# selkies-project/selkies

Hardware: AMD Instinct MI355X
Metric: encoded_fps_1080p60_h264 (higher is better)
Workload: dtype uint8; 1 GPU; model=hipflux h264enc-striped (HIP gfx950), global_batch=1, seq_len=2073600, parallelism=sessions1, resolution=1920x1080, qp=28, content=noise, pipeline=hip-h264, pipeline_depth=2

## Files before the change

native/hip/h264_deblock.hip:

```cpp
#include <hip/hip_runtime.h>

#include <type_traits>

#include "h264_gpu_layout.h"
#include "h264_kernels.h"

namespace hipflux {
namespace h264gpu {

__constant__ uint8_t cDbAlpha[52] = {
    0, 0, 0, 0, 0, 0, 0, 0, 0, 0, 0, 0, 0, 0, 0, 0,
    4, 4, 5, 6, 7, 8, 9, 10, 12, 13, 15, 17, 20, 22, 25, 28,
    32, 36, 40, 45, 50, 56, 63, 71, 80, 90, 101, 113, 127, 144,
    162, 182, 203, 226, 255, 255};
__constant__ uint8_t cDbBeta[52] = {
    0, 0, 0, 0, 0, 0, 0, 0, 0, 0, 0, 0, 0, 0, 0, 0,
    2, 2, 2, 3, 3, 3, 3, 4, 4, 4, 6, 6, 7, 7, 8, 8,
    9, 9, 10, 10, 11, 11, 12, 12, 13, 13, 14, 14, 15, 15,
    16, 16, 17, 17, 18, 18};
__constant__ uint8_t cDbTc0[52][3] = {
    {0,0,0},{0,0,0},{0,0,0},{0,0,0},{0,0,0},{0,0,0},{0,0,0},{0,0,0},
    {0,0,0},{0,0,0},{0,0,0},{0,0,0},{0,0,0},{0,0,0},{0,0,0},{0,0,0},
    {0,0,0},{0,0,1},{0,0,1},{0,0,1},{0,0,1},{0,1,1},{0,1,1},{1,1,1},
    {1,1,1},{1,1,1},{1,1,1},{1,1,2},{1,1,2},{1,1,2},{1,1,2},{1,2,3},
    {1,2,3},{2,2,3},{2,2,4},{2,3,4},{2,3,4},{3,3,5},{3,4,6},{3,4,6},
    {4,5,7},{4,5,8},{5,6,9},{6,7,10},{6,8,11},{7,9,12},{8,10,13},
    {9,12,15},{10,13,17},{11,16,20},{13,18,23},{14,20,25}};

__constant__ int cDbChromaQp[52] = {
    0, 1, 2, 3, 4, 5, 6, 7, 8, 9, 10, 11, 12, 13, 14, 15, 16, 17, 18,
    19, 20, 21, 22, 23, 24, 25, 26, 27, 28, 29, 29, 30, 31, 32, 32, 33,
    34, 34, 35, 35, 36, 36, 37, 37, 37, 38, 38, 38, 39, 39, 39, 39};

__device__ __forceinline__ int db_clip3d(int lo, int hi, int v) {
  return v < lo ? lo : v > hi ? hi : v;
}
__device__ __forceinline__ int db_clip8d(int v) {
  return v < 0 ? 0 : v > 255 ? 255 : v;
}

struct DbInfo {
  int intra;
  int mvx, mvy;
  unsigned nz;
};

__device__ __forceinline__ int db_bs_d(const DbInfo& mp, int pblk,
                                       const DbInfo& mq, int qblk,
                                       bool mb_edge) {
  if (mp.intra || mq.intra) return mb_edge ? 4 : 3;
  if (((mp.nz >> pblk) & 1) || ((mq.nz >> qblk) & 1)) return 2;
  if (abs(mp.mvx - mq.mvx) >= 4 || abs(mp.mvy - mq.mvy) >= 4) return 1;
  return 0;
}

__device__ void db_luma_line(uint8_t* e, int st, int bs, int alpha,
                             int beta, int tc0) {
  const int p0 = e[-st], p1 = e[-2 * st], p2 = e[-3 * st], p3 = e[-4 * st];
  const int q0 = e[0], q1 = e[st], q2 = e[2 * st], q3 = e[3 * st];
  if (abs(p0 - q0) >= alpha || abs(p1 - p0) >= beta ||
      abs(q1 - q0) >= beta)
    return;
  const bool ap = abs(p2 - p0) < beta;
  const bool aq = abs(q2 - q0) < beta;
  if (bs < 4) {
    const int tc = tc0 + (ap ? 1 : 0) + (aq ? 1 : 0);
    const int delta =
        db_clip3d(-tc, tc, ((q0 - p0) * 4 + (p1 - q1) + 4) >> 3);
    e[-st] = (uint8_t)db_clip8d(p0 + delta);
    e[0] = (uint8_t)db_clip8d(q0 - delta);
    if (ap)
      e[-2 * st] = (uint8_t)(p1 + db_clip3d(-tc0, tc0,
                       (p2 + ((p0 + q0 + 1) >> 1) - 2 * p1) >> 1));
    if (aq)
      e[st] = (uint8_t)(q1 + db_clip3d(-tc0, tc0,
                  (q2 + ((p0 + q0 + 1) >> 1) - 2 * q1) >> 1));
  } else {
    const bool small = abs(p0 - q0) < ((alpha >> 2) + 2);
    if (ap && small) {
      e[-st] = (uint8_t)((p2 + 2 * p1 + 2 * p0 + 2 * q0 + q1 + 4) >> 3);
      e[-2 * st] = (uint8_t)((p2 + p1 + p0 + q0 + 2) >> 2);
      e[-3 * st] = (uint8_t)((2 * p3 + 3 * p2 + p1 + p0 + q0 + 4) >> 3);
    } else {
      e[-st] = (uint8_t)((2 * p1 + p0 + q1 + 2) >> 2);
    }
    if (aq && small) {
      e[0] = (uint8_t)((q2 + 2 * q1 + 2 * q0 + 2 * p0 + p1 + 4) >> 3);
      e[st] = (uint8_t)((q2 + q1 + q0 + p0 + 2) >> 2);
      e[2 * st] = (uint8_t)((2 * q3 + 3 * q2 + q1 + q0 + p0 + 4) >> 3);
    } else {
      e[0] = (uint8_t)((2 * q1 + q0 + p1 + 2) >> 2);
    }
  }
}

__device__ void db_chroma_line(uint8_t* e, int st, int bs, int alpha,
                               int beta, int tc0) {
  const int p0 = e[-st], p1 = e[-2 * st];
  const int q0 = e[0], q1 = e[st];
  if (abs(p0 - q0) >= alpha || abs(p1 - p0) >= beta ||
      abs(q1 - q0) >= beta)
    return;
  if (bs < 4) {
    const int tc = tc0 + 1;
    const int delta =
        db_clip3d(-tc, tc, ((q0 - p0) * 4 + (p1 - q1) + 4) >> 3);
    e[-st] = (uint8_t)db_clip8d(p0 + delta);
    e[0] = (uint8_t)db_clip8d(q0 - delta);
  } else {
    e[-st] = (uint8_t)((2 * p1 + p0 + q1 + 2) >> 2);
    e[0] = (uint8_t)((2 * q1 + q0 + p1 + 2) >> 2);
  }
}

struct DbShared {
  uint8_t y[16][kMaxSegMbw * 16];
  uint8_t cb[8][kMaxSegMbw * 8];
  uint8_t cr[8][kMaxSegMbw * 8];
  DbInfo info[kMaxSegMbw];
};

struct DbSharedMono {
  uint8_t y[16][kMaxSegMbw * 16];
  DbInfo info[kMaxSegMbw];
};

template <bool MONO>
__device__ __forceinline__ void deblock_body(
    uint8_t* __restrict__ curY, uint8_t* __restrict__ curCb,
    uint8_t* __restrict__ curCr, int ypitch, int cpitch, int mbw,
    const RowJob& job, const int16_t* __restrict__ levels,
    const int* __restrict__ meta) {
  __shared__ std::conditional_t<MONO, DbSharedMono, DbShared> sh;
  if (job.flags & kJobIdr) {
  }
  const int lane = threadIdx.x;
  const int segw = job.seg_mbw;
  const int y0 = job.mb_row * 16, cy0 = job.mb_row * 8;
  const int px0 = job.mbx0 * 16, cpx0 = job.mbx0 * 8;
  const int wpx = segw * 16, cwpx = segw * 8;

  for (int r = 0; r < 16; ++r)
    for (int x = lane; x < wpx; x += 64)
      sh.y[r][x] = curY[(size_t)(y0 + r) * ypitch + px0 + x];
  if constexpr (!MONO) {
    for (int r = 0; r < 8; ++r)
      for (int x = lane; x < cwpx; x += 64) {
        sh.cb[r][x] = curCb[(size_t)(cy0 + r) * cpitch + cpx0 + x];
        sh.cr[r][x] = curCr[(size_t)(cy0 + r) * cpitch + cpx0 + x];
      }
  }
  for (int m = lane; m < segw; m += 64) {
    const size_t mb = (size_t)job.mb_row * mbw + job.mbx0 + m;
    const int m0 = meta[mb * kMetaPerMb + 0];
    const int m1 = meta[mb * kMetaPerMb + 1];
    const int mode = m0 & 3;
    DbInfo di;
    di.intra = mode == kIntra || (job.flags & kJobIdr);
    di.mvx = mode == kInter ? (int)(short)(m1 & 0xFFFF) : 0;
    di.mvy = mode == kInter ? (m1 >> 16) : 0;
    di.nz = 0;
    if (!MONO && mode == kInter) {
      const int16_t* lv = levels + mb * kLevelsPerMb + kLumaAcOff;
      for (int b = 0; b < 16; ++b) {
        int any = 0;
        for (int i = 0; i < 16; ++i) any |= lv[b * 16 + i] != 0;
        di.nz |= (unsigned)any << b;
      }
    }
    sh.info[m] = di;
  }
  __syncthreads();

  const int qp = db_clip3d(0, 51, job.qp);
  const int qpc = cDbChromaQp[qp];
  const int alpha = cDbAlpha[qp], beta = cDbBeta[qp];
  const int alpha_c = cDbAlpha[qpc], beta_c = cDbBeta[qpc];

  for (int m = 0; m < segw; ++m) {
    const int x0 = m * 16, cx0 = m * 8;
    for (int e = 0; e < 4; ++e) {
      if (lane < 16) {
        if (!(e == 0 && m == 0)) {
          const int pblk = (lane >> 2) * 4 + (e == 0 ? 3 : e - 1);
          const int qblk = (lane >> 2) * 4 + e;
          const DbInfo& mp = e == 0 ? sh.info[m - 1] : sh.info[m];
          const int bs = db_bs_d(mp, pblk, sh.info[m], qblk, e == 0);
          if (bs) {
            const int tc0 = bs < 4 ? cDbTc0[qp][bs - 1] : 0;
            db_luma_line(&sh.y[lane][x0 + e * 4], 1, bs, alpha, beta,
                         tc0);
          }
        }
      } else if constexpr (MONO) {
      } else if (lane < 32 && e < 2) {
        if (!(e == 0 && m == 0)) {
          const int pl = (lane - 16) >> 3, yy = (lane - 16) & 7;
          const int lrow = (yy * 2) >> 2;
          const int pblk = lrow * 4 + (e == 0 ? 3 : 1);
          const int qblk = lrow * 4 + (e == 0 ? 0 : 2);
          const DbInfo& mp = e == 0 ? sh.info[m - 1] : sh.info[m];
          const int bs = db_bs_d(mp, pblk, sh.info[m], qblk, e == 0);
          if (bs) {
            const int tc0 = bs < 4 ? cDbTc0[qpc][bs - 1] : 0;
            uint8_t* base = pl ? &sh.cr[yy][cx0 + e * 4]
                               : &sh.cb[yy][cx0 + e * 4];
            db_chroma_line(base, 1, bs, alpha_c, beta_c, tc0);
          }
        }
      } else if (lane < 32 && e == 2) {
        const int pl = (lane - 16) >> 3, xx = (lane - 16) & 7;
        const int lcol = (xx * 2) >> 2;
        const int pblk = 1 * 4 + lcol;
        const int qblk = 2 * 4 + lcol;
        const int bs = db_bs_d(sh.info[m], pblk, sh.info[m], qblk, false);
        if (bs) {
          const int tc0 = bs < 4 ? cDbTc0[qpc][bs - 1] : 0;
          uint8_t* base = pl ? &sh.cr[4][cx0 + xx] : &sh.cb[4][cx0 + xx];
          db_chroma_line(base, kMaxSegMbw * 8, bs, alpha_c, beta_c, tc0);
        }
      }
      __syncthreads();
    }
    for (int e = 1; e < 4; ++e) {
      if (lane < 16) {
        const int pblk = (e - 1) * 4 + (lane >> 2);
        const int qblk = e * 4 + (lane >> 2);
        const int bs = db_bs_d(sh.info[m], pblk, sh.info[m], qblk, false);
        if (bs) {
          const int tc0 = bs < 4 ? cDbTc0[qp][bs - 1] : 0;
          db_luma_line(&sh.y[e * 4][x0 + lane], kMaxSegMbw * 16, bs,
                       alpha, beta, tc0);
        }
      }
      __syncthreads();
    }
  }

  for (int r = 0; r < 16; ++r)
    for (int x = lane; x < wpx; x += 64)
      curY[(size_t)(y0 + r) * ypitch + px0 + x] = sh.y[r][x];
  if constexpr (!MONO) {
    for (int r = 0; r < 8; ++r)
      for (int x = lane; x < cwpx; x += 64) {
        curCb[(size_t)(cy0 + r) * cpitch + cpx0 + x] = sh.cb[r][x];
        curCr[(size_t)(cy0 + r) * cpitch + cpx0 + x] = sh.cr[r][x];
      }
  }
}

__global__ __launch_bounds__(64) void k_h264_deblock(
    uint8_t* __restrict__ curY, uint8_t* __restrict__ curCb,
    uint8_t* __restrict__ curCr, int ypitch, int cpitch, int mbw,
    const RowJob* __restrict__ jobs, const int16_t* __restrict__ levels,
    const int* __restrict__ meta) {
  const RowJob job = jobs[blockIdx.x];
  deblock_body<false>(curY, curCb, curCr, ypitch, cpitch, mbw, job, levels,
                      meta);
}

__global__ __launch_bounds__(64) void k_h264_deblock_mono(
    uint8_t* __restrict__ cur, size_t plane_stride, int pitch, int mbw,
    const RowJob* __restrict__ jobs, const int* __restrict__ meta) {
  const RowJob job = jobs[blockIdx.x];
  deblock_body<true>(cur + (size_t)job.plane * plane_stride, nullptr,
                     nullptr, pitch, 0, mbw, job, nullptr,
                     meta + (size_t)job.mb_base * kMetaPerMb);
}

void launch_h264_deblock_mono(uint8_t* d_cur, size_t plane_stride, int pitch,
                              int mbw, int n_jobs, const RowJob* d_jobs,
                              const int* d_meta, hipStream_t stream) {
  if (n_jobs == 0) return;
  hipLaunchKernelGGL(k_h264_deblock_mono, dim3(n_jobs), dim3(64), 0, stream,
                     d_cur, plane_stride, pitch, mbw, d_jobs, d_meta);
}

void launch_h264_deblock(uint8_t* d_curY, uint8_t* d_curCb,
                         uint8_t* d_curCr, int ypitch, int cpitch, int mbw,
                         int n_jobs, const RowJob* d_jobs,
                         const int16_t* d_levels, const int* d_meta,
                         hipStream_t stream) {
  if (n_jobs == 0) return;
  hipLaunchKernelGGL(k_h264_deblock, dim3(n_jobs), dim3(64), 0, stream,
                     d_curY, d_curCb, d_curCr, ypitch, cpitch, mbw, d_jobs,
                     d_levels, d_meta);
}

}
}
```

native/hip/h264_kernels.h:

```cpp
#pragma once
#include <hip/hip_runtime.h>

#include <cstdint>

#include "h264_gpu_layout.h"

namespace hipflux {
namespace h264gpu {

void launch_downsample2(const uint8_t* src, int spitch, int sw, int sh,
                        uint8_t* dst, int dpitch, hipStream_t stream);

void launch_h264_me(const uint8_t* srcY, int ypitch, int w, int h,
                    const uint8_t* refY, const uint8_t* srcY2,
                    const uint8_t* refY2, int ypitch2, int mbw, int n_jobs,
                    const RowJob* d_jobs, int* d_meta, hipStream_t stream,
                    bool use_mfma = true);

void launch_h264_rows4(const uint8_t* srcY, const uint8_t* srcCb,
                       const uint8_t* srcCr, int ypitch, int cpitch, int w,
                       int h, const uint8_t* refY, const uint8_t* refCb,
                       const uint8_t* refCr, uint8_t* curY, uint8_t* curCb,
                       uint8_t* curCr, int mbw, int n_jobs,
                       const struct RowJob* d_jobs, int16_t* d_levels,
                       int* d_meta, hipStream_t stream);

void launch_h264_rows(const uint8_t* srcY, const uint8_t* srcCb,
                      const uint8_t* srcCr, int ypitch, int cpitch, int w,
                      int h, const uint8_t* refY, const uint8_t* refCb,
                      const uint8_t* refCr, uint8_t* curY, uint8_t* curCb,
                      uint8_t* curCr, int mbw, int n_jobs,
                      const RowJob* d_jobs, int16_t* d_levels, int* d_meta,
                      hipStream_t stream);

void launch_h264_deblock(uint8_t* d_curY, uint8_t* d_curCb,
                         uint8_t* d_curCr, int ypitch, int cpitch, int mbw,
                         int n_jobs, const RowJob* d_jobs,
                         const int16_t* d_levels, const int* d_meta,
                         hipStream_t stream);

void launch_h264_rows4_mono(const uint8_t* src, const uint8_t* ref,
                            uint8_t* cur, size_t plane_stride, int pitch,
                            int w, int h, int mbw, int n_jobs,
                            const RowJob* d_jobs, int16_t* d_levels,
                            int* d_meta, hipStream_t stream);

void launch_h264_deblock_mono(uint8_t* d_cur, size_t plane_stride, int pitch,
                              int mbw, int n_jobs, const RowJob* d_jobs,
                              const int* d_meta, hipStream_t stream);

void launch_h264_cavlc_mono(const int16_t* d_levels, const int* d_meta,
                            int mbw, int n_jobs, const RowJob* d_jobs,
                            uint32_t* d_stage, int* d_nbits, uint32_t* d_out,
                            int out_stride_words, int* d_out_bits,
                            hipStream_t stream);

void launch_h264_cavlc(const int16_t* d_levels, const int* d_meta, int mbw,
                       int n_jobs, const RowJob* d_jobs, uint32_t* d_stage,
                       int* d_nbits, uint32_t* d_out, int out_stride_words,
                       int* d_out_bits, hipStream_t stream);

}
}
```

native/module.cpp:

```cpp
#include <pybind11/functional.h>
#include <pybind11/numpy.h>
#include <pybind11/pybind11.h>
#include <pybind11/stl.h>

#include "audio.h"
#include "cpu/damage.h"
#include "cpu/h264/cavlc.h"
#include "cpu/h264/encoder.h"
#include "cpu/h264/seg_plan.h"
#include "cpu/hevc/cabac.h"
#include "cpu/hevc/encoder.h"
#include "cpu/opus/celt.h"
#include "cpu/opus/range_coder.h"
#include "cpu/jpeg_enc.h"
#include "cpu/overlay.h"
#include "cpu/scale.h"
#include "engine.h"
#include "frontend_hip.h"
#include <hip/hip_runtime.h>

#include "rccl_comm.h"

namespace py = pybind11;
using namespace hipflux;

namespace hipflux {
int hip_device_count();
}

PYBIND11_MODULE(_native, m) {
  m.doc() = "hipflux: MI355X-native capture+encode engine";

  py::class_<CaptureSettings>(m, "CaptureSettings")
      .def(py::init<>())
      .def_readwrite("capture_width", &CaptureSettings::capture_width)
      .def_readwrite("capture_height", &CaptureSettings::capture_height)
      .def_readwrite("capture_x", &CaptureSettings::capture_x)
      .def_readwrite("capture_y", &CaptureSettings::capture_y)
      .def_readwrite("target_fps", &CaptureSettings::target_fps)
      .def_readwrite("capture_cursor", &CaptureSettings::capture_cursor)
      .def_readwrite("output_mode", &CaptureSettings::output_mode)
      .def_readwrite("capture_scale", &CaptureSettings::capture_scale)
      .def_readwrite("capture_scale_div", &CaptureSettings::capture_scale_div)
      .def_readwrite("pipeline_depth", &CaptureSettings::pipeline_depth)
      .def_readwrite("video_fullframe", &CaptureSettings::video_fullframe)
      .def_readwrite("use_cpu", &CaptureSettings::use_cpu)
      .def_readwrite("gpu_id", &CaptureSettings::gpu_id)
      .def_readwrite("gpu_frontend", &CaptureSettings::gpu_frontend)
      .def_readwrite("video_bitrate_kbps", &CaptureSettings::video_bitrate_kbps)
      .def_readwrite("video_crf", &CaptureSettings::video_crf)
      .def_readwrite("video_cbr_mode", &CaptureSettings::video_cbr_mode)
      .def_readwrite("video_min_qp", &CaptureSettings::video_min_qp)
      .def_readwrite("video_max_qp", &CaptureSettings::video_max_qp)
      .def_readwrite("vbv_multiplier", &CaptureSettings::vbv_multiplier)
      .def_readwrite("keyframe_interval_s", &CaptureSettings::keyframe_interval_s)
      .def_readwrite("video_streaming_mode", &CaptureSettings::video_streaming_mode)
      .def_readwrite("video_deblock", &CaptureSettings::video_deblock)
      .def_readwrite("video_fullcolor", &CaptureSettings::video_fullcolor)
      .def_readwrite("use_paint_over_quality", &CaptureSettings::use_paint_over_quality)
      .def_readwrite("paint_over_trigger_frames", &CaptureSettings::paint_over_trigger_frames)
      .def_readwrite("video_paintover_crf", &CaptureSettings::video_paintover_crf)
      .def_readwrite("video_paintover_burst_frames", &CaptureSettings::video_paintover_burst_frames)
      .def_readwrite("damage_block_threshold", &CaptureSettings::damage_block_threshold)
      .def_readwrite("damage_block_duration", &CaptureSettings::damage_block_duration)
      .def_readwrite("jpeg_quality", &CaptureSettings::jpeg_quality)
      .def_readwrite("jpeg_paintover_quality", &CaptureSettings::jpeg_paintover_quality)
      .def_readwrite("stripe_height", &CaptureSettings::stripe_height)
      .def_readwrite("omit_stripe_headers", &CaptureSettings::omit_stripe_headers)
      .def_readwrite("watermark_path", &CaptureSettings::watermark_path)
      .def_readwrite("watermark_location", &CaptureSettings::watermark_location)
      .def_readwrite("capture_backend", &CaptureSettings::capture_backend)
      .def_readwrite("display", &CaptureSettings::display)
      .def_readwrite("recording_path", &CaptureSettings::recording_path)
      .def_readwrite("debug_logging", &CaptureSettings::debug_logging);

  py::class_<ScreenCapture>(m, "ScreenCapture")
      .def(py::init<>())
      .def(
          "start_capture",
          [](ScreenCapture& self, py::function cb, const CaptureSettings& s) {
            {
              py::gil_scoped_release rel;
              self.stop_capture();
            }
            self.clear_callback();
            StripeCallback native_cb = [cb](const EncodedStripe& st) {
              py::gil_scoped_acquire gil;
              try {
                py::bytes data(reinterpret_cast<const char*>(st.data),
                               st.size);
                cb(data, st.frame_id, st.y, st.width, st.height,
                   st.is_keyframe, st.capture_ts_ms, st.encode_done_ms,
                   static_cast<int>(st.type));
              } catch (py::error_already_set& e) {
                e.discard_as_unraisable("hipflux stripe callback");
              }
            };
            py::gil_scoped_release rel;
            self.start_capture(std::move(native_cb), s);
          },
          py::arg("callback"), py::arg("settings"),
          "Start the native capture+encode thread. callback(data, frame_id, "
          "y, width, height, is_keyframe, capture_ts_ms, encode_done_ms, "
          "stripe_type) runs on the native thread.")
      .def("stop_capture", &ScreenCapture::stop_capture,
           py::call_guard<py::gil_scoped_release>())
      .def(
          "set_cursor_callback",
          [](ScreenCapture& self, py::function cb) {
            self.clear_cursor_callback();
            self.set_cursor_callback(
                [cb](int w, int h, int hx, int hy, const uint32_t* argb,
                     size_t n) {
                  py::gil_scoped_acquire gil;
                  try {
                    cb(w, h, hx, hy,
                       py::bytes(reinterpret_cast<const char*>(argb),
                                 n * 4));
                  } catch (py::error_already_set& e) {
                    e.discard_as_unraisable("hipflux cursor callback");
                  }
                });
          },
          "callback(width, height, hot_x, hot_y, argb_bytes) on shape change")
      .def_property_readonly("is_capturing", &ScreenCapture::is_capturing)
      .def("request_idr_frame", &ScreenCapture::request_idr_frame)
      .def("update_framerate", &ScreenCapture::update_framerate)
      .def("update_video_bitrate", &ScreenCapture::update_video_bitrate)
      .def("update_crf", &ScreenCapture::update_crf)
      .def("update_jpeg_quality", &ScreenCapture::update_jpeg_quality)
      .def("update_vbv_multiplier", &ScreenCapture::update_vbv_multiplier)
      .def("update_capture_region", &ScreenCapture::update_capture_region)
      .def_property_readonly("frames_captured", &ScreenCapture::frames_captured)
      .def_property_readonly("frames_encoded", &ScreenCapture::frames_encoded)
      .def_property_readonly("stripes_emitted", &ScreenCapture::stripes_emitted)
      .def_property_readonly("last_encode_ms", &ScreenCapture::last_encode_ms)
      .def_property_readonly("last_frontend_ms",
                             &ScreenCapture::last_frontend_ms)
      .def_property_readonly("pipeline",
                             [](ScreenCapture& s) { return s.pipeline_name(); })
      .def_property_readonly("frontend",
                             [](ScreenCapture& s) { return s.frontend_name(); });

  m.def(
      "jpeg_encode",
      [](py::buffer bgrx, int width, int height, int quality, bool fullcolor) {
        py::buffer_info info = bgrx.request();
        if (info.size < static_cast<ssize_t>(width) * height * 4)
          throw std::runtime_error("buffer too small for WxHx4");
        std::vector<uint8_t> out;
        {
          py::gil_scoped_release rel;
          jpeg_encode_bgrx(static_cast<const uint8_t*>(info.ptr), width * 4,
                           width, height, quality, fullcolor, out);
        }
        return py::bytes(reinterpret_cast<const char*>(out.data()),
                         out.size());
      },
      py::arg("bgrx"), py::arg("width"), py::arg("height"),
      py::arg("quality") = 80, py::arg("fullcolor") = false,
      "Encode a BGRX buffer as baseline JPEG (CPU reference path).");

  m.def(
      "_jpeg_encode_restart",
      [](py::buffer bgrx, int width, int height, int quality,
         bool fullcolor) {
        py::buffer_info info = bgrx.request();
        std::vector<uint8_t> out;
        {
          py::gil_scoped_release rel;
          jpeg_encode_bgrx(static_cast<const uint8_t*>(info.ptr), width * 4,
                           width, height, quality, fullcolor, out, true);
        }
        return py::bytes(reinterpret_cast<const char*>(out.data()),
                         out.size());
      },
      py::arg("bgrx"), py::arg("width"), py::arg("height"),
      py::arg("quality") = 80, py::arg("fullcolor") = false,
      "Test hook: restart-row JPEG framing (the GPU entropy structure).");

  struct PyH264 {
    h264::StripeEncoder enc;
    int w, h, ypitch, cpitch;
    bool fullcolor;
    std::vector<uint8_t> yuv;
    PyH264(int width, int height, bool deblock, bool fc)
        : enc(width, height, deblock, fc), w(width), h(height),
          fullcolor(fc) {
      ypitch = (w + 15) & ~15;
      cpitch = fullcolor ? ypitch : ypitch / 2;
      int yh = (h + 15) & ~15;
      yuv.resize(static_cast<size_t>(ypitch) * yh * (fullcolor ? 3 : 2) *
                 (fullcolor ? 1 : 3) / (fullcolor ? 1 : 4));
    }
  };
  py::class_<PyH264>(m, "H264Encoder")
      .def(py::init<int, int, bool, bool>(), py::arg("width"),
           py::arg("height"), py::arg("deblock") = true,
           py::arg("fullcolor") = false)
      .def(
          "encode",
          [](PyH264& self, py::buffer bgrx, int qp, bool idr) {
            py::buffer_info info = bgrx.request();
            if (info.size < static_cast<ssize_t>(self.w) * self.h * 4)
              throw std::runtime_error("buffer too small");
            std::vector<uint8_t> out;
            h264::EncodeStats st;
            {
              py::gil_scoped_release rel;
              uint8_t* y = self.yuv.data();
              int yh = (self.h + 15) & ~15;
              uint8_t* cb = y + static_cast<size_t>(self.ypitch) * yh;
              uint8_t* cr = cb + static_cast<size_t>(self.cpitch) *
                                     (self.fullcolor ? yh : yh / 2);
              if (self.fullcolor)
                h264::bgrx_to_yuv444(static_cast<const uint8_t*>(info.ptr),
                                     self.w * 4, self.w, self.h, y, cb, cr,
                                     self.ypitch);
              else
                h264::bgrx_to_yuv420(static_cast<const uint8_t*>(info.ptr),
                                     self.w * 4, self.w, self.h, y,
                                     self.ypitch, cb, cr, self.cpitch);
              self.enc.encode_frame(y, self.ypitch, cb, cr, self.cpitch, qp,
                                    idr, out, &st);
            }
            py::dict d;
            d["data"] = py::bytes(reinterpret_cast<const char*>(out.data()),
                                  out.size());
            d["is_idr"] = st.is_idr;
            d["mb_intra"] = st.mb_intra;
            d["mb_inter"] = st.mb_inter;
            d["mb_skip"] = st.mb_skip;
            return d;
          },
          py::arg("bgrx"), py::arg("qp") = 26, py::arg("idr") = false)
      .def(
          "encode_yuv",
          [](PyH264& self, py::buffer ybuf, py::buffer cbbuf, py::buffer crbuf,
             int qp, bool idr) {
            auto yi = ybuf.request(), cbi = cbbuf.request(),
                 cri = crbuf.request();
            std::vector<uint8_t> out;
            h264::EncodeStats st;
            {
              py::gil_scoped_release rel;
              self.enc.encode_frame(static_cast<const uint8_t*>(yi.ptr),
                                    self.w, static_cast<const uint8_t*>(cbi.ptr),
                                    static_cast<const uint8_t*>(cri.ptr),
                                    (self.w + 1) / 2, qp, idr, out, &st);
            }
            return py::bytes(reinterpret_cast<const char*>(out.data()),
                             out.size());
          },
          py::arg("y"), py::arg("cb"), py::arg("cr"), py::arg("qp") = 26,
          py::arg("idr") = false,
          "Encode from tightly-packed YUV420 planes (pitch = width).")
      .def("recon",
           [](PyH264& self) {
             int yh = (self.h + 15) & ~15;
             int ch = self.fullcolor ? yh : yh / 2;
             py::bytes y(reinterpret_cast<const char*>(self.enc.recon_y()),
                         static_cast<size_t>(self.enc.recon_ypitch()) * yh);
             py::bytes cb(reinterpret_cast<const char*>(self.enc.recon_cb()),
                          static_cast<size_t>(self.enc.recon_cpitch()) * ch);
             py::bytes cr(reinterpret_cast<const char*>(self.enc.recon_cr()),
                          static_cast<size_t>(self.enc.recon_cpitch()) * ch);
             return py::make_tuple(y, cb, cr, self.enc.recon_ypitch(),
                                   self.enc.recon_cpitch());
           });

  struct PyHevc {
    hevc::StripeEncoder enc;
    int w, h, ypitch, cpitch;
    bool fullcolor;
    std::vector<uint8_t> yuv;
    PyHevc(int width, int height, int slices_per_row, bool fc)
        : enc(width, height, slices_per_row, fc), w(width), h(height),
          fullcolor(fc) {
      ypitch = (width + 15) & ~15;
      cpitch = fc ? ypitch : ypitch / 2;
      int yh = (height + 15) & ~15;
      yuv.resize(fc ? static_cast<size_t>(ypitch) * yh * 3
                    : static_cast<size_t>(ypitch) * yh * 3 / 2);
    }
  };
  py::class_<PyHevc>(m, "HevcEncoder")
      .def(py::init<int, int, int, bool>(), py::arg("width"),
           py::arg("height"), py::arg("slices_per_row") = 1,
           py::arg("fullcolor") = false)
      .def(
          "encode",
          [](PyHevc& self, py::buffer bgrx, int qp) {
            py::buffer_info info = bgrx.request();
            if (info.size < static_cast<ssize_t>(self.w) * self.h * 4)
              throw std::runtime_error("buffer too small");
            std::vector<uint8_t> out;
            hevc::EncodeStats st;
            {
              py::gil_scoped_release rel;
              uint8_t* y = self.yuv.data();
              int yh = (self.h + 15) & ~15;
              uint8_t* cb = y + static_cast<size_t>(self.ypitch) * yh;
              uint8_t* cr = cb + static_cast<size_t>(self.cpitch) *
                                     (self.fullcolor ? yh : yh / 2);
              if (self.fullcolor)
                h264::bgrx_to_yuv444(static_cast<const uint8_t*>(info.ptr),
                                     self.w * 4, self.w, self.h, y, cb, cr,
                                     self.ypitch);
              else
                h264::bgrx_to_yuv420(static_cast<const uint8_t*>(info.ptr),
                                     self.w * 4, self.w, self.h, y,
                                     self.ypitch, cb, cr, self.cpitch);
              self.enc.encode_frame(y, self.ypitch, cb, cr, self.cpitch, qp,
                                    out, &st);
            }
            py::dict d;
            d["data"] = py::bytes(reinterpret_cast<const char*>(out.data()),
                                  out.size());
            d["qp"] = st.frame_qp;
            d["ctus"] = st.ctu_count;
            return d;
          },
          py::arg("bgrx"), py::arg("qp") = 30)
      .def("recon", [](PyHevc& self) {
        int yh = (self.h + 15) & ~15;
        int yp = self.enc.recon_ypitch(), cp = self.enc.recon_cpitch();
        int chh = self.fullcolor ? yh : yh / 2;
        py::bytes y(reinterpret_cast<const char*>(self.enc.recon_y()),
                    static_cast<size_t>(yp) * yh);
        py::bytes cb(reinterpret_cast<const char*>(self.enc.recon_cb()),
                     static_cast<size_t>(cp) * chh);
        py::bytes cr(reinterpret_cast<const char*>(self.enc.recon_cr()),
                     static_cast<size_t>(cp) * chh);
        return py::make_tuple(y, cb, cr, yp, cp);
      });

  m.def(
      "_hevc_cabac_encode",
      [](const std::vector<std::tuple<int, int, int>>& ops, int qp) {
        std::vector<uint8_t> bytes;
        hevc::CabacEncoder cab(bytes);
        hevc::ContextBank bank;
        bank.init(qp);
        for (const auto& op : ops) {
          int kind = std::get<0>(op), ctx = std::get<1>(op),
              bin = std::get<2>(op);
          if (kind == 0)
            cab.encode_bin(bank.ctx[ctx % hevc::kNumContexts], bin);
          else if (kind == 1)
            cab.encode_bypass(bin);
          else
            cab.encode_terminate(bin);
        }
        auto tail = cab.finish();
        return py::make_tuple(
            py::bytes(reinterpret_cast<const char*>(bytes.data()),
                      bytes.size()),
            tail.bits, tail.nbits);
      },
      py::arg("ops"), py::arg("qp") = 30);

  py::class_<opus::CeltEncoder>(m, "OpusEncoder")
      .def(py::init<int>(), py::arg("bitrate_bps") = 96000)
      .def("set_bitrate", &opus::CeltEncoder::set_bitrate)
      .def(
          "encode",
          [](opus::CeltEncoder& e, py::buffer pcm, int channels) {
            py::buffer_info info = pcm.request();
            if (info.size <
                static_cast<ssize_t>(opus::kFrameSamples) * channels)
              throw std::runtime_error("need 960 frames of s16 PCM");
            std::vector<uint8_t> out;
            {
              py::gil_scoped_release rel;
              out = e.encode_frame(
                  static_cast<const int16_t*>(info.ptr), channels);
            }
            return py::bytes(reinterpret_cast<const char*>(out.data()),
                             out.size());
          },
          py::arg("pcm"), py::arg("channels") = 2);

  m.def("_opus_range_encode",
        [](const std::vector<std::tuple<int, int, int>>& ops,
           size_t capacity) {
          opus::RangeEncoder ec(capacity);
          static const uint8_t icdf4[4] = {200, 120, 40, 0};
          for (const auto& op : ops) {
            int kind = std::get<0>(op), a = std::get<1>(op),
                b = std::get<2>(op);
            if (kind == 0)
              ec.enc_bit_logp(a, static_cast<unsigned>(b));
            else if (kind == 1)
              ec.enc_uint(static_cast<uint32_t>(a),
                          static_cast<uint32_t>(b));
            else if (kind == 2)
              ec.enc_bits(static_cast<uint32_t>(a),
                          static_cast<unsigned>(b));
            else
              ec.enc_icdf(a % 4, icdf4, 8);
          }
          ec.done();
          auto s = ec.stream();
          return py::make_tuple(
              py::bytes(reinterpret_cast<const char*>(s.data()),
                        s.size()),
              ec.error());
        });

  py::class_<TileComm>(m, "TileComm")
      .def(py::init<int, int, const std::string&, int>(), py::arg("rank"),
           py::arg("world"), py::arg("uid"), py::arg("device") = 0)
      .def_static("make_uid",
                  [] { return py::bytes(TileComm::make_uid()); })
      .def_property_readonly("rank", &TileComm::rank)
      .def_property_readonly("world", &TileComm::world)
      .def(
          "exchange",
          [](TileComm& c, uintptr_t src_dev, size_t bytes, int schedule) {
            py::gil_scoped_release rel;
            return c.exchange(src_dev, bytes, schedule);
          },
          py::arg("src_dev"), py::arg("bytes"), py::arg("schedule") = 1,
          "All-gather this rank's device payload to every rank; "
          "schedule 0 = ring (bulk), 1 = one-hop p2p (latency). "
          "Returns ms.")
      .def(
          "exchange_host",
          [](TileComm& c, py::bytes payload, int schedule) {
            std::string s = payload;
            void* d = nullptr;
            if (hipMalloc(&d, s.size()) != hipSuccess)
              throw std::runtime_error("alloc failed");
            (void)hipMemcpy(d, s.data(), s.size(), hipMemcpyHostToDevice);
            double ms;
            {
              py::gil_scoped_release rel;
              ms = c.exchange(reinterpret_cast<uintptr_t>(d), s.size(),
                              schedule);
            }
            (void)hipFree(d);
            return ms;
          },
          py::arg("payload"), py::arg("schedule") = 1,
          "Upload host bytes and exchange (tests).")
      .def("gathered",
           [](TileComm& c, int rank, size_t bytes) {
             auto v = c.gathered(rank, bytes);
             return py::bytes(reinterpret_cast<const char*>(v.data()),
                              v.size());
           })
      .def(
          "broadcast",
          [](TileComm& c, uintptr_t buf, size_t bytes, int root) {
            py::gil_scoped_release rel;
            return c.broadcast(buf, bytes, root);
          },
          py::arg("buf_dev"), py::arg("bytes"), py::arg("root") = 0,
          "Broadcast a reference-frame buffer from root. Returns ms.");

  m.def(
      "bgrx_to_yuv420",
      [](py::buffer bgrx, int width, int height) {
        py::buffer_info info = bgrx.request();
        int cw = (width + 1) / 2, ch = (height + 1) / 2;
        std::vector<uint8_t> y(static_cast<size_t>(width) * height),
            cb(static_cast<size_t>(cw) * ch), cr(static_cast<size_t>(cw) * ch);
        h264::bgrx_to_yuv420(static_cast<const uint8_t*>(info.ptr), width * 4,
                             width, height, y.data(), width, cb.data(),
                             cr.data(), cw);
        return py::make_tuple(
            py::bytes(reinterpret_cast<char*>(y.data()), y.size()),
            py::bytes(reinterpret_cast<char*>(cb.data()), cb.size()),
            py::bytes(reinterpret_cast<char*>(cr.data()), cr.size()));
      },
      py::arg("bgrx"), py::arg("width"), py::arg("height"));

  m.def(
      "_pipeline_encode",
      [](const std::string& kind, py::list frames, int w, int h, int qp,
         int stripe_h, int output_mode, bool dump, bool fullcolor,
         int pipeline_depth, py::object encode_mask) -> py::object {
        const size_t n_stripes =
            stripe_h > 0 ? static_cast<size_t>((h + stripe_h - 1) / stripe_h)
                         : 0;
        std::vector<std::vector<bool>> mask;
        if (!encode_mask.is_none()) {
          if (!py::isinstance<py::list>(encode_mask))
            throw py::value_error("encode_mask must be a list of lists");
          py::list ml = encode_mask.cast<py::list>();
          if (ml.size() != frames.size())
            throw py::value_error("encode_mask needs one entry per frame");
          for (py::handle fm : ml) {
            if (!py::isinstance<py::list>(fm))
              throw py::value_error("encode_mask must be a list of lists");
            py::list fl = py::reinterpret_borrow<py::list>(fm);
            if (fl.size() != n_stripes)
              throw py::value_error(
                  "encode_mask entry needs one bool per stripe");
            std::vector<bool> row;
            for (py::handle b : fl) row.push_back(b.cast<bool>());
            mask.push_back(std::move(row));
          }
        }
        CaptureSettings s;
        s.capture_width = w;
        s.capture_height = h;
        s.output_mode = output_mode;
        s.stripe_height = stripe_h;
        s.video_crf = qp;
        s.jpeg_quality = qp;
        s.video_fullcolor = fullcolor;
        s.use_cpu = kind == "cpu";
        s.gpu_id = kind == "cpu" ? -1 : 0;
        std::unique_ptr<EncodePipeline> p;
        if (kind == "gpu") {
          p = make_hip_pipeline(s);
          if (!p) throw std::runtime_error("no HIP pipeline available");
        } else {
          p = output_mode == 1   ? make_cpu_h264_pipeline(s)
              : output_mode == 2 ? make_cpu_hevc_pipeline(s)
                                 : make_cpu_jpeg_pipeline(s);
        }
        p->set_pipeline_depth(pipeline_depth);
        std::vector<py::list> per_frame(frames.size());
        auto sink = [&](EncodedStripe& st) {
          per_frame[st.frame_id].append(py::make_tuple(
              py::bytes(reinterpret_cast<const char*>(st.data), st.size),
              st.y, st.height, st.is_keyframe));
        };
        py::list result;
        for (size_t i = 0; i < frames.size(); ++i) {
          py::buffer buf = frames[i].cast<py::buffer>();
          py::buffer_info info = buf.request();
          if (info.size < static_cast<ssize_t>(w) * h * 4)
            throw std::runtime_error("frame buffer too small");
          RawFrame f;
          f.data = static_cast<const uint8_t*>(info.ptr);
          f.width = w;
          f.height = h;
          f.stride = w * 4;
          f.ts_ms = now_ms();
          FrameContext ctx;
          ctx.frame_id = static_cast<uint32_t>(i);
          ctx.idr = (i == 0);
          ctx.crf = qp;
          ctx.jpeg_quality = qp;
          for (int y = 0; y < h; y += stripe_h) {
            StripeJob j;
            j.y0 = y;
            j.y1 = std::min(y + stripe_h, h);
            j.encode = mask.empty() || mask[i][ctx.stripes.size()];
            ctx.stripes.push_back(j);
          }
          p->encode_frame(f, ctx, sink);
        }
        p->flush(sink);
        for (auto& fo : per_frame) result.append(fo);
        if (dump) {
          EncodePipeline::DebugDump d;
          if (!p->debug_dump(d))
            throw std::runtime_error("pipeline has no debug_dump");
          py::dict dd;
          dd["w"] = d.w;
          dd["h"] = d.h;
          dd["ypitch"] = d.ypitch;
          dd["cpitch"] = d.cpitch;
          dd["y"] = py::bytes(reinterpret_cast<char*>(d.y.data()),
                              d.y.size());
          dd["cb"] = py::bytes(reinterpret_cast<char*>(d.cb.data()),
                               d.cb.size());
          dd["cr"] = py::bytes(reinterpret_cast<char*>(d.cr.data()),
                               d.cr.size());
          dd["levels"] = py::bytes(
              reinterpret_cast<char*>(d.levels.data()),
              d.levels.size() * sizeof(int16_t));
          dd["meta"] = py::bytes(reinterpret_cast<char*>(d.meta.data()),
                                 d.meta.size() * sizeof(int));
          return py::object(py::make_tuple(result, dd));
        }
        return py::object(result);
      },
      py::arg("kind"), py::arg("frames"), py::arg("w"), py::arg("h"),
      py::arg("qp") = 26, py::arg("stripe_h") = 64,
      py::arg("output_mode") = 1, py::arg("dump") = false,
      py::arg("fullcolor") = false, py::arg("pipeline_depth") = 1,
      py::arg("encode_mask") = py::none(),
      "Test hook: run frames through a named encode pipeline. "
      "encode_mask[frame][stripe] (optional) gates which stripes encode.");

  struct BenchPipeline {
    std::unique_ptr<EncodePipeline> p;
    int w, h, qp, stripe_h;
    uint32_t frame_id = 0;
    long last_frame_id = -1;
    void* d_boundary = nullptr;
    size_t boundary_cap = 0;
    bool keep_stripes = false;
    long kept_frame_id = -1;
    std::vector<std::pair<int, std::string>> kept;
    void note(const EncodedStripe& st) {
      if (!keep_stripes) return;
      if (static_cast<long>(st.frame_id) != kept_frame_id) {
        kept.clear();
        kept_frame_id = st.frame_id;
      }
      kept.emplace_back(
          st.y, std::string(reinterpret_cast<const char*>(st.data), st.size));
    }
    BenchPipeline(const std::string& kind, int width, int height, int qp_,
                  int stripe, int output_mode, int gpu_id,
                  int pipeline_depth, bool fullcolor)
        : w(width), h(height), qp(qp_), stripe_h(stripe) {
      CaptureSettings s;
      s.capture_width = w;
      s.capture_height = h;
      s.output_mode = output_mode;
      s.stripe_height = stripe_h;
      s.video_crf = qp;
      s.jpeg_quality = qp;
      s.gpu_id = gpu_id;
      s.video_fullcolor = fullcolor;
      s.use_cpu = kind == "cpu";
      if (kind == "gpu") {
        p = make_hip_pipeline(s);
        if (!p) throw std::runtime_error("no HIP pipeline available");
      } else {
        p = output_mode == 1   ? make_cpu_h264_pipeline(s)
            : output_mode == 2 ? make_cpu_hevc_pipeline(s)
                               : make_cpu_jpeg_pipeline(s);
      }
      p->set_pipeline_depth(pipeline_depth);
    }
  };
  py::class_<BenchPipeline>(m, "BenchPipeline")
      .def(py::init<const std::string&, int, int, int, int, int, int,
                    int, bool>(),
           py::arg("kind"), py::arg("width"), py::arg("height"),
           py::arg("qp") = 28, py::arg("stripe_height") = 64,
           py::arg("output_mode") = 1, py::arg("gpu_id") = 0,
           py::arg("pipeline_depth") = 1, py::arg("fullcolor") = false)
      .def_property_readonly("pipeline",
                             [](BenchPipeline& b) { return b.p->name(); })
      .def_readonly("last_frame_id", &BenchPipeline::last_frame_id)
      .def_readwrite("keep_stripes", &BenchPipeline::keep_stripes,
                     "When true, encode()/flush() keep a copy of the newest "
                     "emitted frame's stripes for kept_stripes().")
      .def(
          "kept_stripes",
          [](BenchPipeline& b) {
            py::list out;
            for (auto& s : b.kept)
              out.append(py::make_tuple(s.first, py::bytes(s.second)));
            return py::make_tuple(b.kept_frame_id, out);
          },
          "(frame_id, [(y, payload bytes), ...]) of the newest frame "
          "emitted while keep_stripes was set.")
      .def(
          "boundary_dev",
          [](BenchPipeline& b, int rows) {
            void* y = nullptr;
            int ypitch = 0, height = 0;
            if (!b.p->recon_dev(&y, &ypitch, &height)) {
              return py::make_tuple(static_cast<uintptr_t>(0),
                                    static_cast<size_t>(0));
            }
            rows = std::min(rows, height / 2);
            size_t need = static_cast<size_t>(ypitch) * rows * 2;
            if (b.boundary_cap < need) {
              if (b.d_boundary) (void)hipFree(b.d_boundary);
              if (hipMalloc(&b.d_boundary, need) != hipSuccess)
                throw std::runtime_error("boundary alloc failed");
              b.boundary_cap = need;
            }
            auto* dst = static_cast<uint8_t*>(b.d_boundary);
            auto* srcy = static_cast<uint8_t*>(y);
            size_t half = static_cast<size_t>(ypitch) * rows;
            if (hipMemcpy(dst, srcy, half, hipMemcpyDeviceToDevice) !=
                    hipSuccess ||
                hipMemcpy(dst + half,
                          srcy + static_cast<size_t>(ypitch) *
                                     (height - rows),
                          half, hipMemcpyDeviceToDevice) != hipSuccess)
              throw std::runtime_error("boundary pack failed");
            return py::make_tuple(
                reinterpret_cast<uintptr_t>(b.d_boundary),
                static_cast<size_t>(need));
          },
          py::arg("rows") = 16,
          "Pack top+bottom recon rows into a device buffer; returns "
          "(dev_ptr, nbytes) for TileComm.exchange.")
      .def(
          "resize",
          [](BenchPipeline& b, int w, int h) {
            b.w = w;
            b.h = h;
          },
          py::arg("w"), py::arg("h"),
          "Change frame dimensions (next encode reallocates; an "
          "in-flight pipelined frame is dropped, streams restart IDR).")
      .def(
          "flush",
          [](BenchPipeline& b) {
            size_t total = 0;
            int stripes = 0;
            long done = -1;
            {
              py::gil_scoped_release rel;
              b.p->flush([&](EncodedStripe& st) {
                total += st.size;
                ++stripes;
                done = st.frame_id;
                b.note(st);
              });
            }
            b.last_frame_id = done;
            return py::make_tuple(total, stripes);
          },
          "Emit any pipelined frame still in flight (depth 2); returns "
          "(bitstream_bytes, stripes).")
      .def(
          "encode",
          [](BenchPipeline& b, py::buffer bgrx, bool idr) {
            py::buffer_info info = bgrx.request();
            if (info.size < static_cast<ssize_t>(b.w) * b.h * 4)
              throw std::runtime_error("frame buffer too small");
            size_t total = 0;
            int stripes = 0;
            {
              py::gil_scoped_release rel;
              RawFrame f;
              f.data = static_cast<const uint8_t*>(info.ptr);
              f.width = b.w;
              f.height = b.h;
              f.stride = b.w * 4;
              f.ts_ms = now_ms();
              FrameContext ctx;
              ctx.frame_id = b.frame_id++;
              ctx.idr = idr;
              ctx.crf = b.qp;
              ctx.jpeg_quality = b.qp;
              for (int y = 0; y < b.h; y += b.stripe_h) {
                StripeJob j;
                j.y0 = y;
                j.y1 = std::min(y + b.stripe_h, b.h);
                j.encode = true;
                ctx.stripes.push_back(j);
              }
              long done = -1;
              b.p->encode_frame(f, ctx, [&](EncodedStripe& st) {
                total += st.size;
                ++stripes;
                done = st.frame_id;
                b.note(st);
              });
              b.last_frame_id = done;
            }
            return py::make_tuple(total, stripes);
          },
          py::arg("bgrx"), py::arg("idr") = false,
          "Encode one frame; returns (bitstream_bytes, stripes).");

  m.def(
      "_h264_seg_plan",
      [](py::array_t<int> mbw, py::array_t<int> mbh,
         py::array_t<int> override_segs) {
        auto segs = py::vectorize([](int w, int h, int o) {
          return h264::seg_plan(w, h, o).segs;
        });
        auto widest = py::vectorize([](int w, int h, int o) {
          return h264::seg_plan(w, h, o).widest;
        });
        return py::make_tuple(segs(mbw, mbh, override_segs),
                              widest(mbw, mbh, override_segs));
      },
      py::arg("mbw"), py::arg("mbh"), py::arg("override_segs") = 0,
      "Slice plan of the HIP H.264 pipeline -> (slices per MB row, widest "
      "slice in MBs); override_segs < 1 = none. Broadcasts over arrays.");

  m.def(
      "_cavlc_bits",
      [](std::vector<int> zz, int nC) {
        h264::BitWriter bw;
        int tmp[16] = {};
        for (size_t i = 0; i < zz.size() && i < 16; ++i) tmp[i] = zz[i];
        h264::cavlc_residual(bw, tmp, static_cast<int>(zz.size()), nC);
        size_t nbits = bw.bit_count();
        bw.put_bit(1);
        while (bw.bit_count() % 8) bw.put_bit(0);
        std::string s;
        const auto& bytes = bw.bytes();
        for (size_t i = 0; i < nbits; ++i)
          s += ((bytes[i / 8] >> (7 - i % 8)) & 1) ? '1' : '0';
        return s;
      },
      "debug: CAVLC-encode one zigzag block, return bit string");

  py::class_<AudioCaptureSettings>(m, "AudioCaptureSettings")
      .def(py::init<>())
      .def_readwrite("device_name", &AudioCaptureSettings::device_name)
      .def_readwrite("sample_rate", &AudioCaptureSettings::sample_rate)
      .def_readwrite("channels", &AudioCaptureSettings::channels)
      .def_readwrite("codec", &AudioCaptureSettings::codec)
      .def_readwrite("opus_bitrate", &AudioCaptureSettings::opus_bitrate)
      .def_readwrite("frame_duration_ms",
                     &AudioCaptureSettings::frame_duration_ms)
      .def_readwrite("red_distance", &AudioCaptureSettings::red_distance)
      .def_readwrite("omit_audio_header",
                     &AudioCaptureSettings::omit_audio_header)
      .def_readwrite("debug_logging", &AudioCaptureSettings::debug_logging);

  py::class_<AudioCapture>(m, "AudioCapture")
      .def(py::init<>())
      .def(
          "start_capture",
          [](AudioCapture& self, const AudioCaptureSettings& s,
             py::function cb) {
            {
              py::gil_scoped_release rel;
              self.stop_capture();
            }
            self.clear_callback();
            AudioCapture::Callback native = [cb](const AudioFrame& f) {
              py::gil_scoped_acquire gil;
              try {
                cb(py::bytes(reinterpret_cast<const char*>(f.data), f.size),
                   f.pts_ms);
              } catch (py::error_already_set& e) {
                e.discard_as_unraisable("hipflux audio callback");
              }
            };
            py::gil_scoped_release rel;
            self.start_capture(s, std::move(native));
          },
          py::arg("settings"), py::arg("callback"))
      .def("stop_capture", &AudioCapture::stop_capture,
           py::call_guard<py::gil_scoped_release>())
      .def_property_readonly("is_capturing", &AudioCapture::is_capturing)
      .def("update_audio_bitrate", &AudioCapture::update_audio_bitrate);

  py::class_<AudioPlaybackSettings>(m, "AudioPlaybackSettings")
      .def(py::init<>())
      .def_readwrite("sample_rate", &AudioPlaybackSettings::sample_rate)
      .def_readwrite("channels", &AudioPlaybackSettings::channels)
      .def_readwrite("max_buffer_bytes",
                     &AudioPlaybackSettings::max_buffer_bytes);

  py::class_<AudioPlayback>(m, "AudioPlayback")
      .def(py::init<const AudioPlaybackSettings&>())
      .def("write",
           [](AudioPlayback& self, py::bytes data) {
             std::string s = data;
             return self.write(
                 reinterpret_cast<const uint8_t*>(s.data()), s.size());
           })
      .def("read",
           [](AudioPlayback& self, size_t n) {
             std::vector<uint8_t> out(n);
             size_t got = self.read(out.data(), n);
             return py::bytes(reinterpret_cast<char*>(out.data()), got);
           })
      .def_property_readonly("buffered", &AudioPlayback::buffered);

  m.def(
      "_bilinear_downscale",
      [](py::buffer bgrx, int w, int h, float scale) {
        py::buffer_info info = bgrx.request();
        if (info.size < static_cast<ssize_t>(w) * h * 4)
          throw std::runtime_error("buffer too small");
        std::vector<uint8_t> out;
        int ow, oh, ostride;
        bilinear_downscale_bgrx(static_cast<const uint8_t*>(info.ptr),
                                w * 4, w, h, scale, out, ow, oh, ostride);
        return py::make_tuple(
            py::bytes(reinterpret_cast<const char*>(out.data()), out.size()),
            ow, oh);
      },
      py::arg("bgrx"), py::arg("w"), py::arg("h"), py::arg("scale"),
      "Test hook: exact fixed-point bilinear downscale (engine path).");

  py::class_<DamageTracker>(m, "_DamageTracker")
      .def(py::init<>())
      .def("reset", &DamageTracker::reset, py::arg("width"),
           py::arg("height"), py::arg("block") = 16)
      .def(
          "update",
          [](DamageTracker& d, py::buffer cur, int stride, int threshold,
             int duration) {
            py::buffer_info info = cur.request();
            d.update(static_cast<const uint8_t*>(info.ptr), stride, threshold,
                     duration);
          },
          py::arg("cur"), py::arg("stride"), py::arg("threshold"),
          py::arg("duration"))
      .def(
          "apply_dirty",
          [](DamageTracker& d, py::object flags, int duration) {
            if (flags.is_none()) {
              d.apply_dirty(nullptr, duration);
              return;
            }
            py::buffer_info info = flags.cast<py::buffer>().request();
            if (info.size * info.itemsize <
                static_cast<ssize_t>(d.blocks_x()) * d.blocks_y())
              throw std::runtime_error("flag map too small");
            d.apply_dirty(static_cast<const uint8_t*>(info.ptr), duration);
          },
          py::arg("flags"), py::arg("duration"),
          "flags: blocks_x*blocks_y bytes (nonzero = changed), or None = "
          "everything changed")
      .def("ages",
           [](const DamageTracker& d) {
             return py::array_t<uint16_t>(d.ages().size(), d.ages().data());
           })
      .def_property_readonly("blocks_x", &DamageTracker::blocks_x)
      .def_property_readonly("blocks_y", &DamageTracker::blocks_y)
      .def("consecutive_still_frames",
           &DamageTracker::consecutive_still_frames);

  struct FrontHook {
    int w, h;
    float scale;
    int div;
    Watermark wm;
    int wm_location = 0;
    CursorImage cursor;
    DamageTracker damage;
    int dmg_w = 0, dmg_h = 0;
    bool dmg_on = true;

    FrontHook(int width, int height, float s, int d)
        : w(width), h(height), scale(std::min(1.0f, std::max(0.25f, s))),
          div(std::min(4, std::max(1, d))) {}

    RawFrame frame_of(const py::buffer_info& info, int stride, int width,
                      int height) const {
      RawFrame f;
      f.width = width > 0 ? width : w;
      f.height = height > 0 ? height : h;
      f.stride = stride > 0 ? stride : f.width * 4;
      f.data = static_cast<const uint8_t*>(info.ptr);
      if (f.stride < f.width * 4 || f.stride % 4 ||
          info.size * info.itemsize <
              static_cast<ssize_t>(f.stride) * (f.height - 1) + f.width * 4)
        throw std::runtime_error("buffer too small for the frame geometry");
      return f;
    }
    bool take_cursor(const py::object& c) {
      if (c.is_none()) return false;
      py::tuple t = c.cast<py::tuple>();
      py::buffer_info bi = t[0].cast<py::buffer>().request();
      const int cw = t[1].cast<int>(), ch = t[2].cast<int>();
      if (cw <= 0 || ch <= 0 ||
          bi.size * bi.itemsize < static_cast<ssize_t>(cw) * ch * 4)
        throw std::runtime_error("cursor image too small");
      std::vector<uint32_t> px(static_cast<size_t>(cw) * ch);
      std::memcpy(px.data(), bi.ptr, px.size() * 4);
      if (px != cursor.argb || cw != cursor.width || ch != cursor.height) {
        cursor.argb = std::move(px);
        ++cursor.serial;
      }
      cursor.width = cw;
      cursor.height = ch;
      cursor.x = t[3].cast<int>();
      cursor.y = t[4].cast<int>();
      return true;
    }
    void set_watermark(py::buffer bgra, int ww, int wh, int location) {
      py::buffer_info info = bgra.request();
      if (ww <= 0 || wh <= 0 ||
          info.size * info.itemsize < static_cast<ssize_t>(ww) * wh * 4)
        throw std::runtime_error("watermark image too small");
      wm.w = ww;
      wm.h = wh;
      const uint8_t* p = static_cast<const uint8_t*>(info.ptr);
      wm.bgra.assign(p, p + static_cast<size_t>(ww) * wh * 4);
      wm_location = location;
    }
    bool track(int ow, int oh, bool on) {
      if (ow == dmg_w && oh == dmg_h && on == dmg_on) return false;
      damage.reset(ow, oh);
      dmg_w = ow;
      dmg_h = oh;
      dmg_on = on;
      return true;
    }
    py::dict result(const std::vector<uint8_t>& tight, int ow, int oh) const {
      py::dict d;
      d["frame"] = py::bytes(reinterpret_cast<const char*>(tight.data()),
                             tight.size());
      d["w"] = ow;
      d["h"] = oh;
      d["ages"] =
          py::array_t<uint16_t>(damage.ages().size(), damage.ages().data());
      d["still_frames"] = damage.consecutive_still_frames();
      return d;
    }
  };

  struct PyGpuFrontEnd : FrontHook {
    std::unique_ptr<GpuFrontEnd> fe;
    PyGpuFrontEnd(int width, int height, float s, int d, int gpu_id,
                  bool pin_source)
        : FrontHook(width, height, s, d),
          fe(make_gpu_frontend(width, height, s, d, gpu_id, pin_source)) {}
  };
  py::class_<PyGpuFrontEnd>(m, "GpuFrontEnd")
      .def(py::init<int, int, float, int, int, bool>(), py::arg("width"),
           py::arg("height"), py::arg("scale") = 1.0f,
           py::arg("scale_div") = 1, py::arg("gpu_id") = 0,
           py::arg("pin_source") = false,
           "Device capture front end. pin_source=True page-locks the frame "
           "buffers it is given in place: pass only buffers that outlive "
           "this object.")
      .def(
          "set_watermark",
          [](PyGpuFrontEnd& self, py::buffer bgra, int ww, int wh,
             int location) {
            self.set_watermark(bgra, ww, wh, location);
            self.fe->set_watermark(self.wm.bgra.data(), ww, wh);
          },
          py::arg("bgra"), py::arg("w"), py::arg("h"), py::arg("location"))
      .def("set_timing",
           [](PyGpuFrontEnd& self, bool on) { self.fe->set_timing(on); })
      .def("last_stage_ms",
           [](PyGpuFrontEnd& self) {
             GpuFrontEnd::StageMs t = self.fe->last_stage_ms();
             py::dict d;
             d["h2d"] = t.h2d;
             d["overlay"] = t.overlay;
             d["scale"] = t.scale;
             d["damage"] = t.damage;
             return d;
           })
      .def(
          "process",
          [](PyGpuFrontEnd& self, py::buffer bgrx, int stride,
             py::object cursor, uint64_t frame_idx, int threshold,
             int duration, bool damage, int width, int height,
             bool download) {
            py::buffer_info info = bgrx.request();
            RawFrame f = self.frame_of(info, stride, width, height);
            GpuFrontEnd::Overlay ov;
            if (self.wm.w > 0) {
              ov.wm_location = self.wm_location;
              ov.wm_frame = frame_idx;
            }
            if (self.take_cursor(cursor)) ov.cursor = &self.cursor;
            GpuFrontEnd::Result r;
            std::vector<uint8_t> tight;
            {
              py::gil_scoped_release rel;
              r = self.fe->process(f, ov, threshold, damage);
              if (self.track(r.width, r.height, damage)) r.flags = nullptr;
              if (damage) self.damage.apply_dirty(r.flags, duration);
              if (download) self.fe->download(tight);
            }
            return self.result(tight, r.width, r.height);
          },
          py::arg("bgrx"), py::arg("stride") = 0,
          py::arg("cursor") = py::none(), py::arg("frame_idx") = 0,
          py::arg("threshold") = 15, py::arg("duration") = 30,
          py::arg("damage") = true, py::arg("width") = 0,
          py::arg("height") = 0, py::arg("download") = true,
          "One frame through upload, overlay, downscale and block diff on "
          "the GPU -> {frame, w, h, ages, still_frames}. cursor = (argb, cw, "
          "ch, x, y); width/height 0 = the constructor's; download=False "
          "leaves frame empty (timing).");

  struct PyCpuFrontEnd : FrontHook {
    std::vector<uint8_t> scratch, scaled, tight;
    PyCpuFrontEnd(int width, int height, float s, int d, int, bool)
        : FrontHook(width, height, s, d) {}
  };
  py::class_<PyCpuFrontEnd>(m, "_frontend_cpu")
      .def(py::init<int, int, float, int, int, bool>(), py::arg("width"),
           py::arg("height"), py::arg("scale") = 1.0f,
           py::arg("scale_div") = 1, py::arg("gpu_id") = 0,
           py::arg("pin_source") = false,
           "Host twin of GpuFrontEnd: the engine's host code "
           "(cpu/overlay.h, cpu/scale.h, DamageTracker::update).")
      .def("set_watermark", &PyCpuFrontEnd::set_watermark, py::arg("bgra"),
           py::arg("w"), py::arg("h"), py::arg("location"))
      .def(
          "process",
          [](PyCpuFrontEnd& self, py::buffer bgrx, int stride,
             py::object cursor, uint64_t frame_idx, int threshold,
             int duration, bool damage, int width, int height,
             bool download) {
            py::buffer_info info = bgrx.request();
            RawFrame f = self.frame_of(info, stride, width, height);
            const bool have_cursor = self.take_cursor(cursor);
            int ow = f.width, oh = f.height;
            {
              py::gil_scoped_release rel;
              const uint8_t* data = f.data;
              if (self.wm.w > 0 || have_cursor) {
                const size_t bytes =
                    static_cast<size_t>(f.stride) * (f.height - 1) +
                    static_cast<size_t>(f.width) * 4;
                self.scratch.assign(data, data + bytes);
                if (self.wm.w > 0)
                  self.wm.composite(self.scratch.data(), f.width, f.height,
                                    f.stride, self.wm_location, frame_idx);
                if (have_cursor)
                  composite_cursor(self.scratch.data(), f.width, f.height,
                                   f.stride, self.cursor.argb.data(),
                                   self.cursor.width, self.cursor.height,
                                   self.cursor.x, self.cursor.y);
                data = self.scratch.data();
              }
              int ostride = f.stride;
              if (self.scale < 0.9999f) {
                bilinear_downscale_bgrx(data, f.stride, f.width, f.height,
                                        self.scale, self.scaled, ow, oh,
                                        ostride);
                data = self.scaled.data();
              } else if (self.div > 1) {
                box_downscale_bgrx(data, f.stride, f.width, f.height,
                                   self.div, self.scaled, ow, oh, ostride);
                data = self.scaled.data();
              }
              self.track(ow, oh, damage);
              if (damage) self.damage.update(data, ostride, threshold, duration);
              self.tight.clear();
              if (download) {
                self.tight.resize(static_cast<size_t>(ow) * oh * 4);
                for (int y = 0; y < oh; ++y)
                  std::memcpy(self.tight.data() + static_cast<size_t>(y) * ow * 4,
                              data + static_cast<size_t>(y) * ostride,
                              static_cast<size_t>(ow) * 4);
              }
            }
            return self.result(self.tight, ow, oh);
          },
          py::arg("bgrx"), py::arg("stride") = 0,
          py::arg("cursor") = py::none(), py::arg("frame_idx") = 0,
          py::arg("threshold") = 15, py::arg("duration") = 30,
          py::arg("damage") = true, py::arg("width") = 0,
          py::arg("height") = 0, py::arg("download") = true);

  m.def(
      "_d2d_copy_ms",
      [](size_t bytes, int iters) {
        void *a = nullptr, *b = nullptr;
        hipEvent_t e0, e1;
        if (hipMalloc(&a, bytes) != hipSuccess ||
            hipMalloc(&b, bytes) != hipSuccess) {
          (void)hipFree(a);
          throw std::runtime_error("hipMalloc failed");
        }
        (void)hipEventCreate(&e0);
        (void)hipEventCreate(&e1);
        (void)hipMemcpyAsync(b, a, bytes, hipMemcpyDeviceToDevice, nullptr);
        (void)hipEventRecord(e0, nullptr);
        for (int i = 0; i < iters; ++i)
          (void)hipMemcpyAsync(b, a, bytes, hipMemcpyDeviceToDevice, nullptr);
        (void)hipEventRecord(e1, nullptr);
        (void)hipEventSynchronize(e1);
        float ms = 0;
        (void)hipEventElapsedTime(&ms, e0, e1);
        (void)hipEventDestroy(e0);
        (void)hipEventDestroy(e1);
        (void)hipFree(a);
        (void)hipFree(b);
        return ms / std::max(1, iters);
      },
      py::arg("bytes"), py::arg("iters") = 20,
      "Mean ms of one device-to-device copy of `bytes` (tools).");

  m.def(
      "screenshot",
      [](const std::string& backend, const std::string& display, int w,
         int h) {
        std::unique_ptr<FrameSource> src;
        {
          py::gil_scoped_release rel;
          if (backend == "x11" || (backend == "auto" && !display.empty()))
            src = make_x11_source(display, 0, 0, w, h);
          if (!src) {
            std::string pattern = "desktop";
            auto pos = backend.find(':');
            if (pos != std::string::npos) pattern = backend.substr(pos + 1);
            src = make_synthetic_source(w > 0 ? w : 1920, h > 0 ? h : 1080,
                                        pattern);
          }
        }
        RawFrame f;
        if (!src->acquire(f)) throw std::runtime_error("capture failed");
        std::vector<uint8_t> out(static_cast<size_t>(f.width) * f.height * 4);
        for (int y = 0; y < f.height; ++y)
          std::memcpy(out.data() + static_cast<size_t>(y) * f.width * 4,
                      f.data + static_cast<size_t>(y) * f.stride,
                      static_cast<size_t>(f.width) * 4);
        return py::make_tuple(
            py::bytes(reinterpret_cast<char*>(out.data()), out.size()),
            f.width, f.height);
      },
      py::arg("backend") = "auto", py::arg("display") = "",
      py::arg("w") = 0, py::arg("h") = 0,
      "One-shot framebuffer grab -> (bgrx, w, h).");

  m.def("hip_device_count", &hip_device_count,
        "Number of usable HIP devices (0 on CPU-only hosts).");
  m.attr("HEVC_BYTES_PER_CTU") = hip_hevc_bytes_per_ctu(false);
  m.attr("HEVC_FULLCOLOR_BYTES_PER_CTU") = hip_hevc_bytes_per_ctu(true);
  m.def("__version__", [] { return "0.1.0"; });
}
```

native/pipeline_hip_h264.cpp:

```cpp
#include <cstdio>
#include <cstdlib>

#include "cpu/h264/gpu_entropy.h"
#include "cpu/h264/headers.h"
#include "cpu/h264/seg_plan.h"
#include "engine.h"
#include "hip/h264_kernels.h"
#include "hip/jpeg_kernels.h"
#include "hip_host.h"
#include "thread_pool.h"

namespace hipflux {
namespace {

class HipH264Pipeline : public EncodePipeline {
 public:
  explicit HipH264Pipeline(const CaptureSettings& s)
      : settings_(s), pool_(encode_pool_threads()), dev_(s.gpu_id) {
    stripe_h_ = std::max(16, s.stripe_height & ~15);
    alloc_for(s.capture_width, s.capture_height);
  }

  struct Out {
    std::vector<uint8_t> header;
    std::vector<std::vector<uint8_t>> rows;
    int plane_slices = 0;
    std::vector<uint8_t> bytes;
    h264::GpuStripeParams p{};
    int y0 = 0, h = 0;
    bool idr = false;
  };
  struct Pending {
    bool active = false;
    int par = 0;
    int n_jobs = 0;
    int copy_words = 0;
    double ts_ms = 0;
    uint32_t frame_id = 0;
    std::vector<Out> outs;
    std::vector<std::pair<int, int>> job_map;
  };

  Pending submit_frame(const RawFrame& frame, const FrameContext& ctx) {
    if (frame.width != w_ || frame.height != h_)
      alloc_for(frame.width, frame.height);
    const int par = parity_;
    const int qp = std::min(51, std::max(0, ctx.crf));

    const size_t frame_bytes = static_cast<size_t>(frame.stride) * frame.height;
    if (frame.dev)
      HIP_CHECK(hipMemcpyAsync(d_frame_[par], frame.dev, frame_bytes,
                               hipMemcpyDeviceToDevice, up_stream_));
    else
      HIP_CHECK(hipMemcpyAsync(d_frame_[par],
                               uploader_.source(frame.data, frame_bytes),
                               frame_bytes, hipMemcpyHostToDevice,
                               up_stream_));
    HIP_CHECK(hipEventRecord(ev_h2d_[par], up_stream_));
    HIP_CHECK(hipStreamWaitEvent(rows_stream_, ev_h2d_[par], 0));
    launch_bgrx_to_planes(d_frame_[par], w_, h_, frame.stride / 4, d_srcY_,
                          d_srcCb_, d_srcCr_, ypitch_, cpitch_, fc_,
                          rows_stream_);

    struct SJob {
      int idx;
      int y0, y1;
      bool idr;
      uint32_t frame_num, idr_pic_id;
    };
    std::vector<SJob> sjobs;
    int n_jobs = 0;
    for (size_t i = 0; i < ctx.stripes.size(); ++i) {
      const auto& st = ctx.stripes[i];
      if (!st.encode) continue;
      auto& state = stripes_[st.y0 / stripe_h_];
      bool idr = ctx.idr || state.need_idr;
      if (idr) {
        state.frame_num = 0;
        ++state.idr_pic_id;
        state.need_idr = false;
      }
      SJob sj{static_cast<int>(st.y0 / stripe_h_), st.y0, st.y1, idr,
              state.frame_num, state.idr_pic_id};
      ++state.frame_num;
      sjobs.push_back(sj);
      int row0 = st.y0 / 16;
      int rows = (std::min(st.y1, mbh_ * 16) - st.y0 + 15) / 16;
      int sy0 = st.y0, sy1 = (row0 + rows) * 16;
      for (int pl = 0; pl < planes_; ++pl) {
        for (int r = 0; r < rows; ++r) {
          int x = 0;
          for (int sg = 0; sg < segs_; ++sg) {
            int segw = std::min(seg_w0_, mbw_ - x);
            h_jobs_[par][n_jobs].mb_row = row0 + r;
            h_jobs_[par][n_jobs].qp = qp;
            h_jobs_[par][n_jobs].flags =
                (sj.idr ? h264gpu::kJobIdr : 0) |
                (settings_.video_deblock ? h264gpu::kJobDeblock : 0) |
                (fc_ ? h264gpu::kJobMono : 0);
            h_jobs_[par][n_jobs].plane = pl;
            h_jobs_[par][n_jobs].mb_base = pl * mbw_ * mbh_;
            h_jobs_[par][n_jobs].stripe_y0 = sy0;
            h_jobs_[par][n_jobs].stripe_y1 = sy1;
            h_jobs_[par][n_jobs].first_mb = r * mbw_ + x;
            h_jobs_[par][n_jobs].frame_num = static_cast<int>(sj.frame_num);
            h_jobs_[par][n_jobs].idr_pic_id = static_cast<int>(sj.idr_pic_id);
            h_jobs_[par][n_jobs].mbx0 = x;
            h_jobs_[par][n_jobs].seg_mbw = segw;
            x += segw;
            ++n_jobs;
          }
        }
      }
    }
    if (n_jobs == 0) return Pending{};
    parity_ ^= 1;

    const int me_jobs = n_jobs / planes_;
    if (fc_) {
      int at[3] = {n_jobs, n_jobs + me_jobs, n_jobs + 2 * me_jobs};
      for (int j = 0; j < n_jobs; ++j)
        h_jobs_[par][at[h_jobs_[par][j].plane]++] = h_jobs_[par][j];
    }
    HIP_CHECK(hipMemcpyAsync(d_jobs_[par], h_jobs_[par],
                             sizeof(h264gpu::RowJob) * n_jobs *
                                 (fc_ ? 2 : 1),
                             hipMemcpyHostToDevice, rows_stream_));
    HIP_CHECK(hipMemcpyAsync(d_meta_[par], d_meta_[par ^ 1], meta_bytes_,
                             hipMemcpyDeviceToDevice, rows_stream_));
    for (int pl = 0; pl < planes_; ++pl) {
      const uint8_t* src = d_srcY_ + pl * plane_stride_;
      const uint8_t* ref = d_refY_ + pl * plane_stride_;
      uint8_t* src2 = d_srcY2_ + pl * pyr_stride_;
      uint8_t* ref2 = d_refY2_ + pl * pyr_stride_;
      if (!ctx.idr) {
        h264gpu::launch_downsample2(src, ypitch_, ypitch_, mbh_ * 16,
                                    d_mip1_, ypitch_ / 2, rows_stream_);
        h264gpu::launch_downsample2(d_mip1_, ypitch_ / 2, ypitch_ / 2,
                                    mbh_ * 8, src2, ypitch_ / 4,
                                    rows_stream_);
        h264gpu::launch_downsample2(ref, ypitch_, ypitch_, mbh_ * 16,
                                    d_mip1_, ypitch_ / 2, rows_stream_);
        h264gpu::launch_downsample2(d_mip1_, ypitch_ / 2, ypitch_ / 2,
                                    mbh_ * 8, ref2, ypitch_ / 4,
                                    rows_stream_);
      }
      h264gpu::launch_h264_me(
          src, ypitch_, w_, h_, ref, src2, ref2, ypitch_ / 4, mbw_, me_jobs,
          d_jobs_[par] + (fc_ ? n_jobs + pl * me_jobs : 0),
          d_meta_[par] + pl * n_mb_ * h264gpu::kMetaPerMb, rows_stream_);
    }

    if (fc_)
      h264gpu::launch_h264_rows4_mono(
          d_srcY_, d_refY_, d_curY_, plane_stride_, ypitch_, w_, h_, mbw_,
          n_jobs, d_jobs_[par], d_levels_[par], d_meta_[par], rows_stream_);
    else
      (rows_v1_ ? h264gpu::launch_h264_rows : h264gpu::launch_h264_rows4)(
          d_srcY_, d_srcCb_, d_srcCr_, ypitch_, cpitch_, w_, h_, d_refY_,
          d_refCb_, d_refCr_, d_curY_, d_curCb_, d_curCr_, mbw_, n_jobs,
          d_jobs_[par], d_levels_[par], d_meta_[par], rows_stream_);
    if (cpu_entropy_) {
      const int row0 = h_jobs_[par][0].mb_row;
      const int rows = h_jobs_[par][n_jobs - 1].mb_row + 1 - row0;
      const size_t lvl_row = static_cast<size_t>(mbw_) * h264gpu::kLevelsPerMb;
      const size_t meta_row = static_cast<size_t>(mbw_) * h264gpu::kMetaPerMb;
      for (int pl = 0; pl < planes_; ++pl) {
        const size_t lo = (static_cast<size_t>(pl) * mbh_ + row0) * lvl_row;
        const size_t mo = (static_cast<size_t>(pl) * mbh_ + row0) * meta_row;
        HIP_CHECK(hipMemcpyAsync(h_levels_ + lo, d_levels_[par] + lo,
                                 rows * lvl_row * sizeof(int16_t),
                                 hipMemcpyDeviceToHost, rows_stream_));
        HIP_CHECK(hipMemcpyAsync(h_meta_ + mo, d_meta_[par] + mo,
                                 rows * meta_row * sizeof(int),
                                 hipMemcpyDeviceToHost, rows_stream_));
      }
    }
    HIP_CHECK(hipEventRecord(ev_rows_[par], rows_stream_));
    if (settings_.video_deblock) {
      HIP_CHECK(hipStreamWaitEvent(db_stream_, ev_rows_[par], 0));
      if (fc_)
        h264gpu::launch_h264_deblock_mono(d_curY_, plane_stride_, ypitch_,
                                          mbw_, n_jobs, d_jobs_[par],
                                          d_meta_[par], db_stream_);
      else
        h264gpu::launch_h264_deblock(d_curY_, d_curCb_, d_curCr_, ypitch_,
                                     cpitch_, mbw_, n_jobs, d_jobs_[par],
                                     d_levels_[par], d_meta_[par],
                                     db_stream_);
      HIP_CHECK(hipEventRecord(ev_db_[par], db_stream_));
    }
    int copy_words = 0;
    if (!cpu_entropy_) {
      HIP_CHECK(hipStreamWaitEvent(stream_, ev_rows_[par], 0));
      (fc_ ? h264gpu::launch_h264_cavlc_mono : h264gpu::launch_h264_cavlc)(
          d_levels_[par], d_meta_[par], mbw_, n_jobs, d_jobs_[par], d_stage_,
          d_nbits_, d_entout_[par], ent_stride_words_, d_outbits_[par],
          stream_);
      copy_words =
          readback_.read(h_entout_[par], d_entout_[par], n_jobs, stream_);
      HIP_CHECK(hipMemcpyAsync(h_outbits_[par], d_outbits_[par],
                               sizeof(int) * n_jobs, hipMemcpyDeviceToHost,
                               stream_));
    }
    if (settings_.video_deblock)
      HIP_CHECK(hipStreamWaitEvent(rows_stream_, ev_db_[par], 0));
    {
      int span_y0 = -1, span_y1 = -1;
      auto flush_span = [&] {
        if (span_y0 < 0) return;
        int rows16 = (std::min(span_y1, mbh_ * 16) - span_y0 + 15) / 16;
        copy_region(d_refY_, d_curY_, ypitch_, span_y0, rows16 * 16);
        if (fc_) {
          copy_region(d_refCb_, d_curCb_, ypitch_, span_y0, rows16 * 16);
          copy_region(d_refCr_, d_curCr_, ypitch_, span_y0, rows16 * 16);
        } else {
          copy_region(d_refCb_, d_curCb_, cpitch_, span_y0 / 2, rows16 * 8);
          copy_region(d_refCr_, d_curCr_, cpitch_, span_y0 / 2, rows16 * 8);
        }
        span_y0 = span_y1 = -1;
      };
      for (const auto& sj : sjobs) {
        if (span_y1 == sj.y0) {
          span_y1 = sj.y1;
        } else {
          flush_span();
          span_y0 = sj.y0;
          span_y1 = sj.y1;
        }
      }
      flush_span();
    }
    HIP_CHECK(hipEventRecord(ev_done_[par],
                             cpu_entropy_ ? rows_stream_ : stream_));

    Pending pd;
    pd.active = true;
    pd.par = par;
    pd.n_jobs = n_jobs;
    pd.copy_words = copy_words;
    pd.ts_ms = frame.ts_ms;
    pd.frame_id = ctx.frame_id;
    pd.outs.resize(sjobs.size());
    pd.job_map.resize(n_jobs);
    {
      int j = 0;
      for (size_t i = 0; i < sjobs.size(); ++i) {
        const auto& sj = sjobs[i];
        Out& o = pd.outs[i];
        o.y0 = sj.y0;
        o.h = std::min(sj.y1, h_) - sj.y0;
        o.idr = sj.idr;
        h264::GpuStripeParams& p = o.p;
        p.levels = h_levels_;
        p.meta = h_meta_;
        p.mbw = mbw_;
        p.mb_row0 = sj.y0 / 16;
        p.n_mb_rows = (std::min(sj.y1, mbh_ * 16) - sj.y0 + 15) / 16;
        p.width = w_;
        p.height = o.h;
        p.qp = qp;
        p.idr = sj.idr;
        p.deblock = settings_.video_deblock;
        p.frame_num = sj.frame_num;
        p.idr_pic_id = sj.idr_pic_id;
        o.plane_slices = p.n_mb_rows * segs_;
        o.rows.resize(o.plane_slices * planes_);
        if (p.idr) {
          const int smbw = (p.width + 15) / 16;
          if (fc_)
            h264::write_sps_444(o.header, smbw, p.n_mb_rows, p.width,
                                p.height,
                                h264::level_idc_for(smbw, p.n_mb_rows));
          else
            h264::write_sps_nal(o.header, smbw, p.n_mb_rows, p.width,
                                p.height);
          h264::write_pps_nal(o.header);
        }
        for (int r = 0; r < o.plane_slices * planes_; ++r)
          pd.job_map[j++] = {int(i), r};
      }
    }
    return pd;
  }

  void collect_pending(Pending& pd, const Emit& emit) {
    if (!pd.active) return;
    pd.active = false;
    const double c0 = timing_ ? now_us() : 0;
    const int par = pd.par;
    ev_done_[par].sync();
    const double c1 = timing_ ? now_us() : 0;
    if (cpu_entropy_) {
      for (int j = 0; j < pd.n_jobs; ++j) {
        auto [si, sl] = pd.job_map[j];
        auto* dst = &pd.outs[si].rows[sl];
        h264::GpuStripeParams pp = pd.outs[si].p;
        if (fc_) {
          pp.colour_plane = h_jobs_[par][j].plane;
          pp.mb_base = static_cast<size_t>(h_jobs_[par][j].mb_base);
        }
        const int psl = sl % pd.outs[si].plane_slices;
        int r = psl / segs_;
        int mbx0 = h_jobs_[par][j].mbx0, segw = h_jobs_[par][j].seg_mbw;
        bool long_sc = psl == 0;
        pool_.submit([pp, r, mbx0, segw, long_sc, dst] {
          h264::encode_seg_nal_from_gpu(pp, r, mbx0, segw, long_sc, *dst);
        });
      }
      pool_.wait_all();
    } else {
      readback_.settle(
          h_entout_[par], d_entout_[par], pd.n_jobs, pd.copy_words,
          [&](int j) { return (h_outbits_[par][j] + 31) / 32 + 1; },
          [&](int max_words) {
            return std::min(ent_stride_words_, max_words * 2 + 64);
          });
      const int nw = std::min(pool_.size(), pd.n_jobs);
      for (int t = 0; t < nw; ++t) {
        pool_.submit([this, &pd, par, t, nw] {
          for (int j = t; j < pd.n_jobs; j += nw) {
            auto [si, sl] = pd.job_map[j];
            h264::assemble_gpu_row_nal(
                h_entout_[par] + (size_t)j * ent_stride_words_,
                h_outbits_[par][j], pd.outs[si].idr,
                sl % pd.outs[si].plane_slices == 0, pd.outs[si].rows[sl]);
          }
        });
      }
      pool_.wait_all();
    }
    const double c2 = timing_ ? now_us() : 0;
    if (pd.outs.size() > 1) {
      for (auto& o : pd.outs)
        pool_.submit([&o] {
          o.bytes = std::move(o.header);
          size_t total = o.bytes.size();
          for (auto& r : o.rows) total += r.size();
          o.bytes.reserve(total);
          for (auto& r : o.rows)
            o.bytes.insert(o.bytes.end(), r.begin(), r.end());
        });
      pool_.wait_all();
    } else {
      for (auto& o : pd.outs) {
        o.bytes = std::move(o.header);
        for (auto& r : o.rows)
          o.bytes.insert(o.bytes.end(), r.begin(), r.end());
      }
    }
    for (auto& o : pd.outs) {
      if (o.bytes.empty()) continue;
      EncodedStripe s;
      s.type = StripeType::kH264;
      s.data = o.bytes.data();
      s.size = o.bytes.size();
      s.frame_id = pd.frame_id;
      s.capture_ts_ms = pd.ts_ms;
      s.y = o.y0;
      s.width = w_;
      s.height = o.h;
      s.is_keyframe = o.idr;
      emit(s);
    }
    if (timing_ && !cpu_entropy_) {
      tm_sync_ += c1 - c0;
      tm_asm_ += c2 - c1;
      tm_concat_ += now_us() - c2;
    }
  }

  void encode_frame(const RawFrame& frame, const FrameContext& ctx,
                    const Emit& emit) override {
    const double t0 = timing_ ? now_us() : 0;
    Pending cur = submit_frame(frame, ctx);
    const double t1 = timing_ ? now_us() : 0;
    if (!cur.active) {
      collect_pending(prev_, emit);
      return;
    }
    if (depth_ < 2 || cpu_entropy_) {
      collect_pending(cur, emit);
      return;
    }
    collect_pending(prev_, emit);
    const double t2 = timing_ ? now_us() : 0;
    prev_ = std::move(cur);
    ev_h2d_[prev_.par].sync();
    if (timing_) {
      tm_submit_ += t1 - t0;
      tm_collect_ += t2 - t1;
      tm_h2d_ += now_us() - t2;
      if (++tm_n_ == 256) {
        std::fprintf(stderr,
                     "[times us/frame] submit=%.0f collect=%.0f (sync=%.0f "
                     "asm=%.0f concat=%.0f) h2dwait=%.0f\n",
                     tm_submit_ / tm_n_, tm_collect_ / tm_n_,
                     tm_sync_ / tm_n_, tm_asm_ / tm_n_, tm_concat_ / tm_n_,
                     tm_h2d_ / tm_n_);
        tm_submit_ = tm_collect_ = tm_h2d_ = tm_sync_ = tm_asm_ =
            tm_concat_ = 0;
        tm_n_ = 0;
      }
    }
  }

  void flush(const Emit& emit) override { collect_pending(prev_, emit); }

  void set_pipeline_depth(int d) override {
    depth_ = std::max(1, std::min(2, d));
  }

  const char* name() const override { return "hip-h264"; }

  bool recon_dev(void** y, int* ypitch, int* height) override {
    *y = d_refY_;
    *ypitch = ypitch_;
    *height = mbh_ * 16;
    return d_refY_ != nullptr;
  }

  bool debug_dump(DebugDump& d) override {
    stream_.sync();
    rows_stream_.sync();
    d.w = w_;
    d.h = h_;
    d.ypitch = ypitch_;
    d.cpitch = cpitch_;
    size_t ysz = static_cast<size_t>(ypitch_) * mbh_ * 16;
    size_t csz = fc_ ? ysz : static_cast<size_t>(cpitch_) * mbh_ * 8;
    d.y.resize(ysz);
    d.cb.resize(csz);
    d.cr.resize(csz);
    HIP_CHECK(hipMemcpy(d.y.data(), d_refY_, ysz, hipMemcpyDeviceToHost));
    HIP_CHECK(hipMemcpy(d.cb.data(), d_refCb_, csz, hipMemcpyDeviceToHost));
    HIP_CHECK(hipMemcpy(d.cr.data(), d_refCr_, csz, hipMemcpyDeviceToHost));
    size_t nlv = n_mb_ * planes_ * h264gpu::kLevelsPerMb;
    size_t nmt = n_mb_ * planes_ * h264gpu::kMetaPerMb;
    d.levels.resize(nlv);
    d.meta.resize(nmt);
    const int last_par = parity_ ^ 1;
    HIP_CHECK(hipMemcpy(d.levels.data(), d_levels_[last_par],
                        nlv * sizeof(int16_t),
                        hipMemcpyDeviceToHost));
    HIP_CHECK(hipMemcpy(d.meta.data(), d_meta_[last_par],
                        nmt * sizeof(int),
                        hipMemcpyDeviceToHost));
    return true;
  }

 private:
  struct StripeState {
    uint32_t frame_num = 0;
    uint32_t idr_pic_id = 0;
    bool need_idr = true;
  };

  void copy_region(uint8_t* dst, const uint8_t* src, int pitch, int y0,
                   int rows) {
    HIP_CHECK(hipMemcpyAsync(dst + static_cast<size_t>(y0) * pitch,
                             src + static_cast<size_t>(y0) * pitch,
                             static_cast<size_t>(rows) * pitch,
                             hipMemcpyDeviceToDevice, rows_stream_));
  }

  void alloc_for(int w, int h) {
    prev_.active = false;
    stream_.sync();
    up_stream_.sync();
    db_stream_.sync();
    rows_stream_.sync();
    arena_.release();
    w_ = h_ = 0;
    mbw_ = (w + 15) / 16;
    mbh_ = (h + 15) / 16;
    ypitch_ = mbw_ * 16;
    cpitch_ = fc_ ? ypitch_ : mbw_ * 8;
    const size_t ysz = static_cast<size_t>(ypitch_) * mbh_ * 16;
    const size_t csz = static_cast<size_t>(cpitch_) * mbh_ * 8;
    for (int i = 0; i < 2; ++i)
      arena_.dev(d_frame_[i], static_cast<size_t>(w) * h * 4);
    plane_stride_ = fc_ ? ysz : 0;
    if (fc_) {
      arena_.dev(d_srcY_, 3 * ysz);
      arena_.dev(d_refY_, 3 * ysz);
      arena_.dev(d_curY_, 3 * ysz);
      d_srcCb_ = d_srcY_ + ysz;
      d_srcCr_ = d_srcY_ + 2 * ysz;
      d_refCb_ = d_refY_ + ysz;
      d_refCr_ = d_refY_ + 2 * ysz;
      d_curCb_ = d_curY_ + ysz;
      d_curCr_ = d_curY_ + 2 * ysz;
    } else {
      arena_.dev(d_srcY_, ysz);
      arena_.dev(d_srcCb_, csz);
      arena_.dev(d_srcCr_, csz);
      arena_.dev(d_refY_, ysz);
      arena_.dev(d_refCb_, csz);
      arena_.dev(d_refCr_, csz);
      arena_.dev(d_curY_, ysz);
      arena_.dev(d_curCb_, csz);
      arena_.dev(d_curCr_, csz);
    }
    n_mb_ = static_cast<size_t>(mbw_) * mbh_;
    const size_t n_mb = n_mb_ * planes_;
    meta_bytes_ = n_mb * h264gpu::kMetaPerMb * sizeof(int);
    for (int i = 0; i < 2; ++i) {
      arena_.dev(d_levels_[i], n_mb * h264gpu::kLevelsPerMb);
      arena_.dev(d_meta_[i], n_mb * h264gpu::kMetaPerMb);
      HIP_CHECK(hipMemset(d_meta_[i], 0, meta_bytes_));
    }
    arena_.dev(d_mip1_, static_cast<size_t>(ypitch_ / 2) * mbh_ * 8);
    pyr_stride_ = static_cast<size_t>(ypitch_ / 4) * mbh_ * 4;
    arena_.dev(d_srcY2_, pyr_stride_ * planes_);
    arena_.dev(d_refY2_, pyr_stride_ * planes_);
    const char* segs_env = std::getenv("HIPFLUX_SEGS");
    const h264::SegPlan plan = h264::seg_plan(
        mbw_, mbh_, segs_env ? std::atoi(segs_env) : 0, planes_);
    segs_ = plan.segs;
    seg_w0_ = plan.widest;
    const size_t max_jobs = static_cast<size_t>(mbh_) * segs_ * planes_;
    arena_.pinned(h_levels_, n_mb * h264gpu::kLevelsPerMb);
    arena_.pinned(h_meta_, n_mb * h264gpu::kMetaPerMb);
    cpu_entropy_ = std::getenv("HIPFLUX_CPU_ENTROPY") != nullptr;
    const size_t nitems = h264gpu::items_per_row(seg_w0_);
    ent_stride_words_ =
        static_cast<int>(nitems * h264gpu::kStageWordsPerItem);
    readback_.reset(ent_stride_words_, ent_stride_words_);
    arena_.dev(d_stage_, max_jobs * ent_stride_words_);
    arena_.dev(d_nbits_, max_jobs * nitems);
    for (int i = 0; i < 2; ++i) {
      arena_.dev(d_jobs_[i], max_jobs * (fc_ ? 2 : 1));
      arena_.dev(d_entout_[i], max_jobs * ent_stride_words_);
      arena_.dev(d_outbits_[i], max_jobs);
      arena_.pinned(h_jobs_[i], max_jobs * (fc_ ? 2 : 1));
      arena_.pinned(h_entout_[i], max_jobs * ent_stride_words_);
      arena_.pinned(h_outbits_[i], max_jobs);
    }
    stripes_.assign((h + stripe_h_ - 1) / stripe_h_, StripeState{});
    w_ = w;
    h_ = h;
  }

  CaptureSettings settings_;
  ThreadPool pool_;
  UseDevice dev_;
  Arena arena_;
  FrameUploader uploader_;
  Stream stream_, up_stream_, db_stream_, rows_stream_;
  Event ev_done_[2], ev_h2d_[2], ev_rows_[2], ev_db_[2];
  CompactReadback<uint32_t> readback_;
  int stripe_h_ = 64;
  const bool fc_ = settings_.video_fullcolor;
  const int planes_ = fc_ ? 3 : 1;
  size_t plane_stride_ = 0;
  size_t pyr_stride_ = 0;
  size_t n_mb_ = 0;
  int w_ = 0, h_ = 0, mbw_ = 0, mbh_ = 0, ypitch_ = 0, cpitch_ = 0;
  int segs_ = 1, seg_w0_ = 0;
  uint8_t* d_frame_[2] = {nullptr, nullptr};
  uint8_t *d_srcY_ = nullptr, *d_srcCb_ = nullptr,
          *d_srcCr_ = nullptr, *d_refY_ = nullptr, *d_refCb_ = nullptr,
          *d_refCr_ = nullptr, *d_curY_ = nullptr, *d_curCb_ = nullptr,
          *d_curCr_ = nullptr;
  int16_t* d_levels_[2] = {};
  size_t meta_bytes_ = 0;
  uint8_t *d_mip1_ = nullptr, *d_srcY2_ = nullptr, *d_refY2_ = nullptr;
  int* d_meta_[2] = {};
  int16_t* h_levels_ = nullptr;
  int* h_meta_ = nullptr;
  bool cpu_entropy_ = false;
  h264gpu::RowJob* d_jobs_[2] = {nullptr, nullptr};
  h264gpu::RowJob* h_jobs_[2] = {nullptr, nullptr};
  uint32_t* d_stage_ = nullptr;
  int* d_nbits_ = nullptr;
  uint32_t* d_entout_[2] = {nullptr, nullptr};
  int* d_outbits_[2] = {nullptr, nullptr};
  uint32_t* h_entout_[2] = {nullptr, nullptr};
  int* h_outbits_[2] = {nullptr, nullptr};
  int depth_ = 1;
  int parity_ = 0;
  Pending prev_;
  const bool timing_ = std::getenv("HIPFLUX_TIMES") != nullptr;
  double tm_submit_ = 0, tm_collect_ = 0, tm_h2d_ = 0, tm_sync_ = 0,
         tm_asm_ = 0, tm_concat_ = 0;
  int tm_n_ = 0;
  int ent_stride_words_ = 0;
  const bool rows_v1_ = std::getenv("HIPFLUX_ROWS_V1") != nullptr;
  std::vector<StripeState> stripes_;
};

}

std::unique_ptr<EncodePipeline> make_hip_h264_pipeline(
    const CaptureSettings& s) {
  return std::make_unique<HipH264Pipeline>(s);
}

}
```

Before: 2311 frames/s.

## Deblock cur into ref directly on rows stream with packed word tiles

New measurement: 2309 frames/s. Within noise of the previous version (-0.1%).

```diff
diff --git a/native/cpu/h264/deblock_lines.h b/native/cpu/h264/deblock_lines.h
--- /dev/null
+++ b/native/cpu/h264/deblock_lines.h
@@ -0,0 +1,266 @@
+#pragma once
+
+#include <cstdint>
+#include <cstring>
+
+#include "deblock.h"
+
+#ifndef HIPFLUX_HD
+#if defined(__HIP__)
+#define HIPFLUX_HD __host__ __device__
+#else
+#define HIPFLUX_HD
+#endif
+#endif
+
+namespace hipflux {
+namespace h264 {
+
+struct DblParams {
+  int alpha, beta;
+  int tc0_1, tc0_2, tc0_3;
+};
+
+HIPFLUX_HD inline int dbl_abs(int v) { return v < 0 ? -v : v; }
+HIPFLUX_HD inline int dbl_clip3(int lo, int hi, int v) {
+  return v < lo ? lo : v > hi ? hi : v;
+}
+HIPFLUX_HD inline int dbl_tc0(const DblParams t, int bs) {
+  return bs == 1 ? t.tc0_1 : bs == 2 ? t.tc0_2 : t.tc0_3;
+}
+
+HIPFLUX_HD inline bool dbl_active(const DblParams t, int p1, int p0, int q0,
+                                  int q1) {
+  return dbl_abs(p0 - q0) < t.alpha && dbl_abs(p1 - p0) < t.beta &&
+         dbl_abs(q1 - q0) < t.beta;
+}
+
+HIPFLUX_HD inline void dbl_luma_weak(const DblParams t, int tc0, int p2,
+                                     int& p1, int& p0, int& q0, int& q1,
+                                     int q2) {
+  const bool on = dbl_active(t, p1, p0, q0, q1);
+  const bool ap = dbl_abs(p2 - p0) < t.beta;
+  const bool aq = dbl_abs(q2 - q0) < t.beta;
+  const int tc = tc0 + (ap ? 1 : 0) + (aq ? 1 : 0);
+  const int delta =
+      dbl_clip3(-tc, tc, ((q0 - p0) * 4 + (p1 - q1) + 4) >> 3);
+  const int avg = (p0 + q0 + 1) >> 1;
+  const int np1 = p1 + dbl_clip3(-tc0, tc0, (p2 + avg - 2 * p1) >> 1);
+  const int nq1 = q1 + dbl_clip3(-tc0, tc0, (q2 + avg - 2 * q1) >> 1);
+  const int np0 = dbl_clip3(0, 255, p0 + delta);
+  const int nq0 = dbl_clip3(0, 255, q0 - delta);
+  p1 = on && ap ? np1 : p1;
+  q1 = on && aq ? nq1 : q1;
+  p0 = on ? np0 : p0;
+  q0 = on ? nq0 : q0;
+}
+
+HIPFLUX_HD inline void dbl_luma_strong(const DblParams t, int p3, int& p2,
+                                       int& p1, int& p0, int& q0, int& q1,
+                                       int& q2, int q3) {
+  const bool on = dbl_active(t, p1, p0, q0, q1);
+  const bool small = dbl_abs(p0 - q0) < ((t.alpha >> 2) + 2);
+  const bool sp = small && dbl_abs(p2 - p0) < t.beta;
+  const bool sq = small && dbl_abs(q2 - q0) < t.beta;
+  const int np0 = sp ? (p2 + 2 * p1 + 2 * p0 + 2 * q0 + q1 + 4) >> 3
+                     : (2 * p1 + p0 + q1 + 2) >> 2;
+  const int np1 = (p2 + p1 + p0 + q0 + 2) >> 2;
+  const int np2 = (2 * p3 + 3 * p2 + p1 + p0 + q0 + 4) >> 3;
+  const int nq0 = sq ? (q2 + 2 * q1 + 2 * q0 + 2 * p0 + p1 + 4) >> 3
+                     : (2 * q1 + q0 + p1 + 2) >> 2;
+  const int nq1 = (q2 + q1 + q0 + p0 + 2) >> 2;
+  const int nq2 = (2 * q3 + 3 * q2 + q1 + q0 + p0 + 4) >> 3;
+  p0 = on ? np0 : p0;
+  p1 = on && sp ? np1 : p1;
+  p2 = on && sp ? np2 : p2;
+  q0 = on ? nq0 : q0;
+  q1 = on && sq ? nq1 : q1;
+  q2 = on && sq ? nq2 : q2;
+}
+
+HIPFLUX_HD inline void dbl_luma_line(const DblParams t, int bs, int p3,
+                                     int& p2, int& p1, int& p0, int& q0,
+                                     int& q1, int& q2, int q3) {
+  if (bs == 0) return;
+  if (bs < 4)
+    dbl_luma_weak(t, dbl_tc0(t, bs), p2, p1, p0, q0, q1, q2);
+  else
+    dbl_luma_strong(t, p3, p2, p1, p0, q0, q1, q2, q3);
+}
+
+HIPFLUX_HD inline void dbl_chroma_line(const DblParams t, int bs, int p1,
+                                       int& p0, int& q0, int q1) {
+  if (bs == 0) return;
+  const bool on = dbl_active(t, p1, p0, q0, q1);
+  int np0, nq0;
+  if (bs < 4) {
+    const int tc = dbl_tc0(t, bs) + 1;
+    const int delta =
+        dbl_clip3(-tc, tc, ((q0 - p0) * 4 + (p1 - q1) + 4) >> 3);
+    np0 = dbl_clip3(0, 255, p0 + delta);
+    nq0 = dbl_clip3(0, 255, q0 - delta);
+  } else {
+    np0 = (2 * p1 + p0 + q1 + 2) >> 2;
+    nq0 = (2 * q1 + q0 + p1 + 2) >> 2;
+  }
+  p0 = on ? np0 : p0;
+  q0 = on ? nq0 : q0;
+}
+
+
+HIPFLUX_HD inline void dbl_luma_row(const DblParams t, const int bs[4],
+                                    int px[20]) {
+#pragma unroll
+  for (int e = 0; e < 4; ++e) {
+    int* q = px + 4 * e + 4;
+    dbl_luma_line(t, bs[e], q[-4], q[-3], q[-2], q[-1], q[0], q[1], q[2],
+                  q[3]);
+  }
+}
+
+HIPFLUX_HD inline void dbl_luma_col(const DblParams t, const int bs[3],
+                                    int r[16]) {
+#pragma unroll
+  for (int e = 1; e < 4; ++e) {
+    int* q = r + 4 * e;
+    if (bs[e - 1] != 0)
+      dbl_luma_weak(t, dbl_tc0(t, bs[e - 1]), q[-3], q[-2], q[-1], q[0],
+                    q[1], q[2]);
+  }
+}
+
+HIPFLUX_HD inline void dbl_chroma_row(const DblParams t, const int bs[2],
+                                      int px[12]) {
+  dbl_chroma_line(t, bs[0], px[2], px[3], px[4], px[5]);
+  dbl_chroma_line(t, bs[1], px[6], px[7], px[8], px[9]);
+}
+
+HIPFLUX_HD inline void dbl_chroma_col(const DblParams t, int bs, int r[4]) {
+  dbl_chroma_line(t, bs, r[0], r[1], r[2], r[3]);
+}
+
+
+HIPFLUX_HD inline void dbl_unpack4(uint32_t d, int* px) {
+  px[0] = d & 255;
+  px[1] = (d >> 8) & 255;
+  px[2] = (d >> 16) & 255;
+  px[3] = d >> 24;
+}
+HIPFLUX_HD inline uint32_t dbl_pack4(const int* px) {
+  return static_cast<uint32_t>(px[0]) | static_cast<uint32_t>(px[1]) << 8 |
+         static_cast<uint32_t>(px[2]) << 16 |
+         static_cast<uint32_t>(px[3]) << 24;
+}
+
+
+HIPFLUX_HD inline int dbl_bs(const DbMb& mp, int pblk, const DbMb& mq,
+                             int qblk, bool mb_edge) {
+  if (mp.intra || mq.intra) return mb_edge ? 4 : 3;
+  if (((mp.nz >> pblk) & 1) || ((mq.nz >> qblk) & 1)) return 2;
+  if (dbl_abs(mp.mvx - mq.mvx) >= 4 || dbl_abs(mp.mvy - mq.mvy) >= 4)
+    return 1;
+  return 0;
+}
+
+HIPFLUX_HD inline void dbl_bs_words(const DbMb* left, const DbMb& cur,
+                                    uint64_t& v, uint64_t& h) {
+  v = 0;
+  h = 0;
+#pragma unroll
+  for (int g = 0; g < 4; ++g) {
+    if (left)
+      v |= static_cast<uint64_t>(dbl_bs(*left, g * 4 + 3, cur, g * 4, true))
+           << (4 * g);
+#pragma unroll
+    for (int e = 1; e < 4; ++e) {
+      v |= static_cast<uint64_t>(
+               dbl_bs(cur, g * 4 + e - 1, cur, g * 4 + e, false))
+           << (4 * (4 * e + g));
+      h |= static_cast<uint64_t>(
+               dbl_bs(cur, (e - 1) * 4 + g, cur, e * 4 + g, false))
+           << (4 * (4 * (e - 1) + g));
+    }
+  }
+}
+HIPFLUX_HD inline int dbl_bs_v(uint64_t v, int e, int g) {
+  return static_cast<int>(v >> (4 * (4 * e + g))) & 15;
+}
+HIPFLUX_HD inline int dbl_bs_h(uint64_t h, int e, int g) {
+  return static_cast<int>(h >> (4 * (4 * (e - 1) + g))) & 15;
+}
+
+
+inline DblParams dbl_params(int index) {
+  const int i = db_clip3(0, 51, index);
+  return DblParams{kDbAlpha[i], kDbBeta[i], kDbTc0[i][0], kDbTc0[i][1],
+                   kDbTc0[i][2]};
+}
+
+inline void deblock_segment_lines(uint8_t* Y, int ypitch, uint8_t* Cb,
+                                  uint8_t* Cr, int cpitch, int mb_row,
+                                  int mbx0, int segw, const DbMb* mbs,
+                                  int qp, int qpc) {
+  const DblParams ty = dbl_params(qp), tc = dbl_params(qpc);
+  for (int m = 0; m < segw; ++m) {
+    uint64_t bv, bh;
+    dbl_bs_words(m ? &mbs[m - 1] : nullptr, mbs[m], bv, bh);
+    uint8_t* mb = Y + static_cast<size_t>(mb_row) * 16 * ypitch +
+                  (mbx0 + m) * 16;
+    for (int yy = 0; yy < 16; ++yy) {
+      uint8_t* row = mb + static_cast<size_t>(yy) * ypitch;
+      uint32_t d[5] = {0, 0, 0, 0, 0};
+      std::memcpy(d + (m ? 0 : 1), row - (m ? 4 : 0), m ? 20 : 16);
+      int px[20], bs[4];
+      for (int k = 0; k < 5; ++k) dbl_unpack4(d[k], px + 4 * k);
+      for (int e = 0; e < 4; ++e) bs[e] = dbl_bs_v(bv, e, yy >> 2);
+      dbl_luma_row(ty, bs, px);
+      for (int k = 0; k < 5; ++k) d[k] = dbl_pack4(px + 4 * k);
+      std::memcpy(row - (m ? 4 : 0), d + (m ? 0 : 1), m ? 20 : 16);
+    }
+    for (int xx = 0; xx < 16; ++xx) {
+      int r[16] = {}, bs[3];
+      for (int k = 1; k < 15; ++k)
+        r[k] = mb[static_cast<size_t>(k) * ypitch + xx];
+      for (int e = 1; e < 4; ++e) bs[e - 1] = dbl_bs_h(bh, e, xx >> 2);
+      dbl_luma_col(ty, bs, r);
+      for (int k = 2; k < 14; ++k)
+        mb[static_cast<size_t>(k) * ypitch + xx] =
+            static_cast<uint8_t>(r[k]);
+    }
+  }
+  if (Cb == nullptr) return;
+  for (int pl = 0; pl < 2; ++pl) {
+    uint8_t* C = pl ? Cr : Cb;
+    for (int m = 0; m < segw; ++m) {
+      uint64_t bv, bh;
+      dbl_bs_words(m ? &mbs[m - 1] : nullptr, mbs[m], bv, bh);
+      uint8_t* mb = C + static_cast<size_t>(mb_row) * 8 * cpitch +
+                    (mbx0 + m) * 8;
+      for (int yy = 0; yy < 8; ++yy) {
+        uint8_t* row = mb + static_cast<size_t>(yy) * cpitch;
+        uint32_t d[3] = {0, 0, 0};
+        std::memcpy(d + (m ? 0 : 1), row - (m ? 4 : 0), m ? 12 : 8);
+        int px[12];
+        for (int k = 0; k < 3; ++k) dbl_unpack4(d[k], px + 4 * k);
+        const int bs[2] = {dbl_bs_v(bv, 0, yy >> 1),
+                           dbl_bs_v(bv, 2, yy >> 1)};
+        dbl_chroma_row(tc, bs, px);
+        for (int k = 0; k < 3; ++k) d[k] = dbl_pack4(px + 4 * k);
+        std::memcpy(row - (m ? 4 : 0), d + (m ? 0 : 1), m ? 12 : 8);
+      }
+      for (int xx = 0; xx < 8; ++xx) {
+        int r[4];
+        for (int k = 0; k < 4; ++k)
+          r[k] = mb[static_cast<size_t>(k + 2) * cpitch + xx];
+        dbl_chroma_col(tc, dbl_bs_h(bh, 2, xx >> 1), r);
+        mb[static_cast<size_t>(3) * cpitch + xx] =
+            static_cast<uint8_t>(r[1]);
+        mb[static_cast<size_t>(4) * cpitch + xx] =
+            static_cast<uint8_t>(r[2]);
+      }
+    }
+  }
+}
+
+}
+}
diff --git a/native/hip/h264_deblock.hip b/native/hip/h264_deblock.hip
--- a/native/hip/h264_deblock.hip
+++ b/native/hip/h264_deblock.hip
@@ -2,11 +2,15 @@
 
 #include <type_traits>
 
+#include "cpu/h264/deblock_lines.h"
 #include "h264_gpu_layout.h"
 #include "h264_kernels.h"
 
 namespace hipflux {
 namespace h264gpu {
+
+using h264::DblParams;
+using h264::DbMb;
 
 __constant__ uint8_t cDbAlpha[52] = {
     0, 0, 0, 0, 0, 0, 0, 0, 0, 0, 0, 0, 0, 0, 0, 0,
@@ -32,260 +36,316 @@
     19, 20, 21, 22, 23, 24, 25, 26, 27, 28, 29, 29, 30, 31, 32, 32, 33,
     34, 34, 35, 35, 36, 36, 37, 37, 37, 38, 38, 38, 39, 39, 39, 39};
 
-__device__ __forceinline__ int db_clip3d(int lo, int hi, int v) {
-  return v < lo ? lo : v > hi ? hi : v;
-}
-__device__ __forceinline__ int db_clip8d(int v) {
-  return v < 0 ? 0 : v > 255 ? 255 : v;
-}
-
-struct DbInfo {
-  int intra;
-  int mvx, mvy;
-  unsigned nz;
+__device__ __forceinline__ DblParams db_params(int index) {
+  return DblParams{cDbAlpha[index], cDbBeta[index], cDbTc0[index][0],
+                   cDbTc0[index][1], cDbTc0[index][2]};
+}
+
+constexpr int kYStride = kMaxSegMbw * 4 + 1;
+constexpr int kCStride = kMaxSegMbw * 2 + 1;
+
+struct DbInfoShared {
+  uint64_t bv[kMaxSegMbw];
+  uint64_t bh[kMaxSegMbw];
+  int mv[kMaxSegMbw];
+  uint16_t nz[kMaxSegMbw];
+  uint8_t intra[kMaxSegMbw];
+  uint8_t inter[kMaxSegMbw];
 };
 
-__device__ __forceinline__ int db_bs_d(const DbInfo& mp, int pblk,
-                                       const DbInfo& mq, int qblk,
-                                       bool mb_edge) {
-  if (mp.intra || mq.intra) return mb_edge ? 4 : 3;
-  if (((mp.nz >> pblk) & 1) || ((mq.nz >> qblk) & 1)) return 2;
-  if (abs(mp.mvx - mq.mvx) >= 4 || abs(mp.mvy - mq.mvy) >= 4) return 1;
-  return 0;
-}
-
-__device__ void db_luma_line(uint8_t* e, int st, int bs, int alpha,
-                             int beta, int tc0) {
-  const int p0 = e[-st], p1 = e[-2 * st], p2 = e[-3 * st], p3 = e[-4 * st];
-  const int q0 = e[0], q1 = e[st], q2 = e[2 * st], q3 = e[3 * st];
-  if (abs(p0 - q0) >= alpha || abs(p1 - p0) >= beta ||
-      abs(q1 - q0) >= beta)
-    return;
-  const bool ap = abs(p2 - p0) < beta;
-  const bool aq = abs(q2 - q0) < beta;
-  if (bs < 4) {
-    const int tc = tc0 + (ap ? 1 : 0) + (aq ? 1 : 0);
-    const int delta =
-        db_clip3d(-tc, tc, ((q0 - p0) * 4 + (p1 - q1) + 4) >> 3);
-    e[-st] = (uint8_t)db_clip8d(p0 + delta);
-    e[0] = (uint8_t)db_clip8d(q0 - delta);
-    if (ap)
-      e[-2 * st] = (uint8_t)(p1 + db_clip3d(-tc0, tc0,
-                       (p2 + ((p0 + q0 + 1) >> 1) - 2 * p1) >> 1));
-    if (aq)
-      e[st] = (uint8_t)(q1 + db_clip3d(-tc0, tc0,
-                  (q2 + ((p0 + q0 + 1) >> 1) - 2 * q1) >> 1));
-  } else {
-    const bool small = abs(p0 - q0) < ((alpha >> 2) + 2);
-    if (ap && small) {
-      e[-st] = (uint8_t)((p2 + 2 * p1 + 2 * p0 + 2 * q0 + q1 + 4) >> 3);
-      e[-2 * st] = (uint8_t)((p2 + p1 + p0 + q0 + 2) >> 2);
-      e[-3 * st] = (uint8_t)((2 * p3 + 3 * p2 + p1 + p0 + q0 + 4) >> 3);
+struct DbShared {
+  uint32_t y[16 * kYStride];
+  uint32_t c[16 * kCStride];
+  DbInfoShared info;
+};
+
+struct DbSharedMono {
+  uint32_t y[16 * kYStride];
+  DbInfoShared info;
+};
+
+__device__ __forceinline__ uint64_t db_uniform(uint64_t v) {
+  const uint32_t lo =
+      __builtin_amdgcn_readfirstlane(static_cast<uint32_t>(v));
+  const uint32_t hi =
+      __builtin_amdgcn_readfirstlane(static_cast<uint32_t>(v >> 32));
+  return static_cast<uint64_t>(hi) << 32 | lo;
+}
+
+__device__ __forceinline__ void db_wave_sync() {
+  __builtin_amdgcn_fence(__ATOMIC_RELEASE, "wavefront");
+  __builtin_amdgcn_wave_barrier();
+  __builtin_amdgcn_fence(__ATOMIC_ACQUIRE, "wavefront");
+}
+
+__device__ __forceinline__ DbMb db_mb(const DbInfoShared& s, int m) {
+  DbMb d;
+  d.intra = s.intra[m];
+  d.mvx = static_cast<int16_t>(s.mv[m] & 0xFFFF);
+  d.mvy = static_cast<int16_t>(s.mv[m] >> 16);
+  d.nz = s.nz[m];
+  return d;
+}
+
+__device__ __forceinline__ void db_walk_luma(uint32_t* __restrict__ tile,
+                                             const DbInfoShared& info,
+                                             int segw, int lane,
+                                             const DblParams t) {
+  const int g = lane >> 2;
+  for (int m = 0; m < segw; ++m) {
+    const uint64_t bv = db_uniform(info.bv[m]);
+    const uint64_t bh = db_uniform(info.bh[m]);
+    uint32_t* rp = tile + lane * kYStride + 4 * m;
+    int px[20];
+#pragma unroll
+    for (int k = 0; k < 5; ++k) h264::dbl_unpack4(rp[k], px + 4 * k);
+    if (((bv ^ (bv >> 4)) & 0x0FFF0FFF0FFF0FFFull) == 0) {
+      const int bs[4] = {static_cast<int>(bv) & 15,
+                         static_cast<int>(bv >> 16) & 15,
+                         static_cast<int>(bv >> 32) & 15,
+                         static_cast<int>(bv >> 48) & 15};
+      h264::dbl_luma_row(t, bs, px);
     } else {
-      e[-st] = (uint8_t)((2 * p1 + p0 + q1 + 2) >> 2);
-    }
-    if (aq && small) {
-      e[0] = (uint8_t)((q2 + 2 * q1 + 2 * q0 + 2 * p0 + p1 + 4) >> 3);
-      e[st] = (uint8_t)((q2 + q1 + q0 + p0 + 2) >> 2);
-      e[2 * st] = (uint8_t)((2 * q3 + 3 * q2 + q1 + q0 + p0 + 4) >> 3);
+      const int bs[4] = {h264::dbl_bs_v(bv, 0, g), h264::dbl_bs_v(bv, 1, g),
+                         h264::dbl_bs_v(bv, 2, g), h264::dbl_bs_v(bv, 3, g)};
+      h264::dbl_luma_row(t, bs, px);
+    }
+#pragma unroll
+    for (int k = 0; k < 5; ++k) rp[k] = h264::dbl_pack4(px + 4 * k);
+    db_wave_sync();
+    uint8_t* cp = reinterpret_cast<uint8_t*>(tile + 1 + 4 * m) + lane;
+    int r[16];
+    r[0] = r[15] = 0;
+#pragma unroll
+    for (int k = 1; k < 15; ++k) r[k] = cp[k * kYStride * 4];
+    if (((bh ^ (bh >> 4)) & 0x0FFF0FFF0FFFull) == 0) {
+      const int bs[3] = {static_cast<int>(bh) & 15,
+                         static_cast<int>(bh >> 16) & 15,
+                         static_cast<int>(bh >> 32) & 15};
+      h264::dbl_luma_col(t, bs, r);
     } else {
-      e[0] = (uint8_t)((2 * q1 + q0 + p1 + 2) >> 2);
-    }
-  }
-}
-
-__device__ void db_chroma_line(uint8_t* e, int st, int bs, int alpha,
-                               int beta, int tc0) {
-  const int p0 = e[-st], p1 = e[-2 * st];
-  const int q0 = e[0], q1 = e[st];
-  if (abs(p0 - q0) >= alpha || abs(p1 - p0) >= beta ||
-      abs(q1 - q0) >= beta)
-    return;
-  if (bs < 4) {
-    const int tc = tc0 + 1;
-    const int delta =
-        db_clip3d(-tc, tc, ((q0 - p0) * 4 + (p1 - q1) + 4) >> 3);
-    e[-st] = (uint8_t)db_clip8d(p0 + delta);
-    e[0] = (uint8_t)db_clip8d(q0 - delta);
-  } else {
-    e[-st] = (uint8_t)((2 * p1 + p0 + q1 + 2) >> 2);
-    e[0] = (uint8_t)((2 * q1 + q0 + p1 + 2) >> 2);
-  }
-}
-
-struct DbShared {
-  uint8_t y[16][kMaxSegMbw * 16];
-  uint8_t cb[8][kMaxSegMbw * 8];
-  uint8_t cr[8][kMaxSegMbw * 8];
-  DbInfo info[kMaxSegMbw];
-};
-
-struct DbSharedMono {
-  uint8_t y[16][kMaxSegMbw * 16];
-  DbInfo info[kMaxSegMbw];
-};
+      const int bs[3] = {h264::dbl_bs_h(bh, 1, g), h264::dbl_bs_h(bh, 2, g),
+                         h264::dbl_bs_h(bh, 3, g)};
+      h264::dbl_luma_col(t, bs, r);
+    }
+#pragma unroll
+    for (int k = 2; k < 14; ++k)
+      cp[k * kYStride * 4] = static_cast<uint8_t>(r[k]);
+    db_wave_sync();
+  }
+}
+
+__device__ __forceinline__ void db_walk_chroma(uint32_t* __restrict__ tile,
+                                               const DbInfoShared& info,
+                                               int segw, int lane,
+                                               const DblParams t) {
+  const int g = (lane & 7) >> 1;
+  for (int m = 0; m < segw; ++m) {
+    const uint64_t bv = db_uniform(info.bv[m]);
+    const uint64_t bh = db_uniform(info.bh[m]);
+    uint32_t* rp = tile + lane * kCStride + 2 * m;
+    int px[12];
+#pragma unroll
+    for (int k = 0; k < 3; ++k) h264::dbl_unpack4(rp[k], px + 4 * k);
+    if (((bv ^ (bv >> 4)) & 0x00000FFF00000FFFull) == 0) {
+      const int bs[2] = {static_cast<int>(bv) & 15,
+                         static_cast<int>(bv >> 32) & 15};
+      h264::dbl_chroma_row(t, bs, px);
+    } else {
+      const int bs[2] = {h264::dbl_bs_v(bv, 0, g), h264::dbl_bs_v(bv, 2, g)};
+      h264::dbl_chroma_row(t, bs, px);
+    }
+#pragma unroll
+    for (int k = 0; k < 3; ++k) rp[k] = h264::dbl_pack4(px + 4 * k);
+    db_wave_sync();
+    uint8_t* cp =
+        reinterpret_cast<uint8_t*>(tile + (lane & 8) * kCStride + 1 + 2 * m) +
+        (lane & 7);
+    int r[4];
+#pragma unroll
+    for (int k = 0; k < 4; ++k) r[k] = cp[(k + 2) * kCStride * 4];
+    if (((bh ^ (bh >> 4)) & 0x0FFF0000ull) == 0)
+      h264::dbl_chroma_col(t, static_cast<int>(bh >> 16) & 15, r);
+    else
+      h264::dbl_chroma_col(t, h264::dbl_bs_h(bh, 2, g), r);
+    cp[3 * kCStride * 4] = static_cast<uint8_t>(r[1]);
+    cp[4 * kCStride * 4] = static_cast<uint8_t>(r[2]);
+    db_wave_sync();
+  }
+}
 
 template <bool MONO>
 __device__ __forceinline__ void deblock_body(
-    uint8_t* __restrict__ curY, uint8_t* __restrict__ curCb,
-    uint8_t* __restrict__ curCr, int ypitch, int cpitch, int mbw,
-    const RowJob& job, const int16_t* __restrict__ levels,
+    const uint8_t* curY, const uint8_t* curCb, const uint8_t* curCr,
+    uint8_t* refY, uint8_t* refCb, uint8_t* refCr, int ypitch, int cpitch,
+    int mbw, const RowJob& job, const int16_t* __restrict__ levels,
     const int* __restrict__ meta) {
   __shared__ std::conditional_t<MONO, DbSharedMono, DbShared> sh;
-  if (job.flags & kJobIdr) {
-  }
-  const int lane = threadIdx.x;
+  constexpr int kThreads = MONO ? 64 : 128;
+  const int tid = threadIdx.x;
+  const int lane = tid & 63;
+  const int wave = __builtin_amdgcn_readfirstlane(tid >> 6);
   const int segw = job.seg_mbw;
+  const size_t mb0 = (size_t)job.mb_row * mbw + job.mbx0;
   const int y0 = job.mb_row * 16, cy0 = job.mb_row * 8;
   const int px0 = job.mbx0 * 16, cpx0 = job.mbx0 * 8;
-  const int wpx = segw * 16, cwpx = segw * 8;
-
-  for (int r = 0; r < 16; ++r)
-    for (int x = lane; x < wpx; x += 64)
-      sh.y[r][x] = curY[(size_t)(y0 + r) * ypitch + px0 + x];
+  const int rg = lane >> 4, ml = lane & 15;
+
+  if (wave == 0) {
+    for (int r = rg; r < 16; r += 4) {
+      const uint8_t* src = curY + (size_t)(y0 + r) * ypitch + px0;
+      uint32_t* dst = sh.y + r * kYStride + 1;
+      for (int m = ml; m < segw; m += 16) {
+        const uint4 v = *reinterpret_cast<const uint4*>(src + m * 16);
+        dst[4 * m + 0] = v.x;
+        dst[4 * m + 1] = v.y;
+        dst[4 * m + 2] = v.z;
+        dst[4 * m + 3] = v.w;
+      }
+    }
+    if (lane < 16) sh.y[lane * kYStride] = 0;
+  }
   if constexpr (!MONO) {
-    for (int r = 0; r < 8; ++r)
-      for (int x = lane; x < cwpx; x += 64) {
-        sh.cb[r][x] = curCb[(size_t)(cy0 + r) * cpitch + cpx0 + x];
-        sh.cr[r][x] = curCr[(size_t)(cy0 + r) * cpitch + cpx0 + x];
-      }
-  }
-  for (int m = lane; m < segw; m += 64) {
-    const size_t mb = (size_t)job.mb_row * mbw + job.mbx0 + m;
-    const int m0 = meta[mb * kMetaPerMb + 0];
-    const int m1 = meta[mb * kMetaPerMb + 1];
-    const int mode = m0 & 3;
-    DbInfo di;
-    di.intra = mode == kIntra || (job.flags & kJobIdr);
-    di.mvx = mode == kInter ? (int)(short)(m1 & 0xFFFF) : 0;
-    di.mvy = mode == kInter ? (m1 >> 16) : 0;
-    di.nz = 0;
-    if (!MONO && mode == kInter) {
-      const int16_t* lv = levels + mb * kLevelsPerMb + kLumaAcOff;
-      for (int b = 0; b < 16; ++b) {
-        int any = 0;
-        for (int i = 0; i < 16; ++i) any |= lv[b * 16 + i] != 0;
-        di.nz |= (unsigned)any << b;
-      }
-    }
-    sh.info[m] = di;
-  }
-  __syncthreads();
-
-  const int qp = db_clip3d(0, 51, job.qp);
-  const int qpc = cDbChromaQp[qp];
-  const int alpha = cDbAlpha[qp], beta = cDbBeta[qp];
-  const int alpha_c = cDbAlpha[qpc], beta_c = cDbBeta[qpc];
-
-  for (int m = 0; m < segw; ++m) {
-    const int x0 = m * 16, cx0 = m * 8;
-    for (int e = 0; e < 4; ++e) {
-      if (lane < 16) {
-        if (!(e == 0 && m == 0)) {
-          const int pblk = (lane >> 2) * 4 + (e == 0 ? 3 : e - 1);
-          const int qblk = (lane >> 2) * 4 + e;
-          const DbInfo& mp = e == 0 ? sh.info[m - 1] : sh.info[m];
-          const int bs = db_bs_d(mp, pblk, sh.info[m], qblk, e == 0);
-          if (bs) {
-            const int tc0 = bs < 4 ? cDbTc0[qp][bs - 1] : 0;
-            db_luma_line(&sh.y[lane][x0 + e * 4], 1, bs, alpha, beta,
-                         tc0);
-          }
-        }
-      } else if constexpr (MONO) {
-      } else if (lane < 32 && e < 2) {
-        if (!(e == 0 && m == 0)) {
-          const int pl = (lane - 16) >> 3, yy = (lane - 16) & 7;
-          const int lrow = (yy * 2) >> 2;
-          const int pblk = lrow * 4 + (e == 0 ? 3 : 1);
-          const int qblk = lrow * 4 + (e == 0 ? 0 : 2);
-          const DbInfo& mp = e == 0 ? sh.info[m - 1] : sh.info[m];
-          const int bs = db_bs_d(mp, pblk, sh.info[m], qblk, e == 0);
-          if (bs) {
-            const int tc0 = bs < 4 ? cDbTc0[qpc][bs - 1] : 0;
-            uint8_t* base = pl ? &sh.cr[yy][cx0 + e * 4]
-                               : &sh.cb[yy][cx0 + e * 4];
-            db_chroma_line(base, 1, bs, alpha_c, beta_c, tc0);
-          }
-        }
-      } else if (lane < 32 && e == 2) {
-        const int pl = (lane - 16) >> 3, xx = (lane - 16) & 7;
-        const int lcol = (xx * 2) >> 2;
-        const int pblk = 1 * 4 + lcol;
-        const int qblk = 2 * 4 + lcol;
-        const int bs = db_bs_d(sh.info[m], pblk, sh.info[m], qblk, false);
-        if (bs) {
-          const int tc0 = bs < 4 ? cDbTc0[qpc][bs - 1] : 0;
-          uint8_t* base = pl ? &sh.cr[4][cx0 + xx] : &sh.cb[4][cx0 + xx];
-          db_chroma_line(base, kMaxSegMbw * 8, bs, alpha_c, beta_c, tc0);
+    if (wave == 1) {
+      for (int r = rg; r < 16; r += 4) {
+        const uint8_t* src = (r < 8 ? curCb : curCr) +
+                             (size_t)(cy0 + (r & 7)) * cpitch + cpx0;
+        uint32_t* dst = sh.c + r * kCStride + 1;
+        for (int m = ml; m < segw; m += 16) {
+          const uint2 v = *reinterpret_cast<const uint2*>(src + m * 8);
+          dst[2 * m + 0] = v.x;
+          dst[2 * m + 1] = v.y;
         }
       }
-      __syncthreads();
-    }
-    for (int e = 1; e < 4; ++e) {
-      if (lane < 16) {
-        const int pblk = (e - 1) * 4 + (lane >> 2);
-        const int qblk = e * 4 + (lane >> 2);
-        const int bs = db_bs_d(sh.info[m], pblk, sh.info[m], qblk, false);
-        if (bs) {
-          const int tc0 = bs < 4 ? cDbTc0[qp][bs - 1] : 0;
-          db_luma_line(&sh.y[e * 4][x0 + lane], kMaxSegMbw * 16, bs,
-                       alpha, beta, tc0);
-        }
+      if (lane < 16) sh.c[lane * kCStride] = 0;
+    }
+  }
+  for (int m = tid; m < segw; m += kThreads) {
+    const int2 mm =
+        *reinterpret_cast<const int2*>(meta + (mb0 + m) * kMetaPerMb);
+    const int mode = mm.x & 3;
+    sh.info.intra[m] = mode == kIntra || (job.flags & kJobIdr);
+    sh.info.inter[m] = mode == kInter;
+    sh.info.mv[m] = mode == kInter ? mm.y : 0;
+    sh.info.nz[m] = 0;
+  }
+  __syncthreads();
+
+  if constexpr (!MONO) {
+    const int half = lane >> 5, hl = lane & 31;
+    for (int mb = wave * 2; mb < segw; mb += 4) {
+      const int m = mb + half;
+      bool any = false;
+      if (m < segw && sh.info.inter[m]) {
+        const uint4 v = *reinterpret_cast<const uint4*>(
+            levels + (mb0 + m) * kLevelsPerMb + kLumaAcOff + hl * 8);
+        any = (v.x | v.y | v.z | v.w) != 0;
       }
-      __syncthreads();
-    }
-  }
-
-  for (int r = 0; r < 16; ++r)
-    for (int x = lane; x < wpx; x += 64)
-      curY[(size_t)(y0 + r) * ypitch + px0 + x] = sh.y[r][x];
+      const uint64_t bal = __ballot(any);
+      uint32_t b = half ? static_cast<uint32_t>(bal >> 32)
+                        : static_cast<uint32_t>(bal);
+      b = (b | (b >> 1)) & 0x55555555u;
+      b = (b | (b >> 1)) & 0x33333333u;
+      b = (b | (b >> 2)) & 0x0F0F0F0Fu;
+      b = (b | (b >> 4)) & 0x00FF00FFu;
+      b = (b | (b >> 8)) & 0x0000FFFFu;
+      if (hl == 0 && m < segw) sh.info.nz[m] = static_cast<uint16_t>(b);
+    }
+    __syncthreads();
+  }
+
+  for (int m = tid; m < segw; m += kThreads) {
+    const DbMb cur = db_mb(sh.info, m);
+    uint64_t bv, bh;
+    if (m > 0) {
+      const DbMb left = db_mb(sh.info, m - 1);
+      h264::dbl_bs_words(&left, cur, bv, bh);
+    } else {
+      h264::dbl_bs_words(nullptr, cur, bv, bh);
+    }
+    sh.info.bv[m] = bv;
+    sh.info.bh[m] = bh;
+  }
+  __syncthreads();
+
+  const int qp = h264::dbl_clip3(0, 51, job.qp);
+  if (wave == 0) {
+    if (lane < 16) db_walk_luma(sh.y, sh.info, segw, lane, db_params(qp));
+  }
   if constexpr (!MONO) {
-    for (int r = 0; r < 8; ++r)
-      for (int x = lane; x < cwpx; x += 64) {
-        curCb[(size_t)(cy0 + r) * cpitch + cpx0 + x] = sh.cb[r][x];
-        curCr[(size_t)(cy0 + r) * cpitch + cpx0 + x] = sh.cr[r][x];
+    if (wave == 1) {
+      if (lane < 16)
+        db_walk_chroma(sh.c, sh.info, segw, lane,
+                       db_params(cDbChromaQp[qp]));
+    }
+  }
+  db_wave_sync();
+
+  if (wave == 0) {
+    for (int r = rg; r < 16; r += 4) {
+      uint8_t* dst = refY + (size_t)(y0 + r) * ypitch + px0;
+      const uint32_t* src = sh.y + r * kYStride + 1;
+      for (int m = ml; m < segw; m += 16)
+        *reinterpret_cast<uint4*>(dst + m * 16) =
+            make_uint4(src[4 * m], src[4 * m + 1], src[4 * m + 2],
+                       src[4 * m + 3]);
+    }
+  }
+  if constexpr (!MONO) {
+    if (wave == 1) {
+      for (int r = rg; r < 16; r += 4) {
+        uint8_t* dst = (r < 8 ? refCb : refCr) +
+                       (size_t)(cy0 + (r & 7)) * cpitch + cpx0;
+        const uint32_t* src = sh.c + r * kCStride + 1;
+        for (int m = ml; m < segw; m += 16)
+          *reinterpret_cast<uint2*>(dst + m * 8) =
+              make_uint2(src[2 * m], src[2 * m + 1]);
       }
-  }
-}
-
-__global__ __launch_bounds__(64) void k_h264_deblock(
-    uint8_t* __restrict__ curY, uint8_t* __restrict__ curCb,
-    uint8_t* __restrict__ curCr, int ypitch, int cpitch, int mbw,
-    const RowJob* __restrict__ jobs, const int16_t* __restrict__ levels,
+    }
+  }
+}
+
+__global__ __launch_bounds__(128) void k_h264_deblock(
+    const uint8_t* curY, const uint8_t* curCb, const uint8_t* curCr,
+    uint8_t* refY, uint8_t* refCb, uint8_t* refCr, int ypitch, int cpitch,
+    int mbw, const RowJob* __restrict__ jobs,
+    const int16_t* __restrict__ levels, const int* __restrict__ meta) {
+  const RowJob job = jobs[blockIdx.x];
+  deblock_body<false>(curY, curCb, curCr, refY, refCb, refCr, ypitch,
+                      cpitch, mbw, job, levels, meta);
+}
+
+__global__ __launch_bounds__(64) void k_h264_deblock_mono(
+    const uint8_t* cur, uint8_t* ref, size_t plane_stride, int pitch,
+    int mbw, const RowJob* __restrict__ jobs,
     const int* __restrict__ meta) {
   const RowJob job = jobs[blockIdx.x];
-  deblock_body<false>(curY, curCb, curCr, ypitch, cpitch, mbw, job, levels,
-                      meta);
-}
-
-__global__ __launch_bounds__(64) void k_h264_deblock_mono(
-    uint8_t* __restrict__ cur, size_t plane_stride, int pitch, int mbw,
-    const RowJob* __restrict__ jobs, const int* __restrict__ meta) {
-  const RowJob job = jobs[blockIdx.x];
-  deblock_body<true>(cur + (size_t)job.plane * plane_stride, nullptr,
+  const size_t off = (size_t)job.plane * plane_stride;
+  deblock_body<true>(cur + off, nullptr, nullptr, ref + off, nullptr,
                      nullptr, pitch, 0, mbw, job, nullptr,
                      meta + (size_t)job.mb_base * kMetaPerMb);
 }
 
-void launch_h264_deblock_mono(uint8_t* d_cur, size_t plane_stride, int pitch,
-                              int mbw, int n_jobs, const RowJob* d_jobs,
+void launch_h264_deblock_mono(const uint8_t* d_cur, uint8_t* d_ref,
+                              size_t plane_stride, int pitch, int mbw,
+                              int n_jobs, const RowJob* d_jobs,
                               const int* d_meta, hipStream_t stream) {
   if (n_jobs == 0) return;
   hipLaunchKernelGGL(k_h264_deblock_mono, dim3(n_jobs), dim3(64), 0, stream,
-                     d_cur, plane_stride, pitch, mbw, d_jobs, d_meta);
-}
-
-void launch_h264_deblock(uint8_t* d_curY, uint8_t* d_curCb,
-                         uint8_t* d_curCr, int ypitch, int cpitch, int mbw,
-                         int n_jobs, const RowJob* d_jobs,
-                         const int16_t* d_levels, const int* d_meta,
-                         hipStream_t stream) {
+                     d_cur, d_ref, plane_stride, pitch, mbw, d_jobs, d_meta);
+}
+
+void launch_h264_deblock(const uint8_t* d_curY, const uint8_t* d_curCb,
+                         const uint8_t* d_curCr, uint8_t* d_refY,
+                         uint8_t* d_refCb, uint8_t* d_refCr, int ypitch,
+                         int cpitch, int mbw, int n_jobs,
+                         const RowJob* d_jobs, const int16_t* d_levels,
+                         const int* d_meta, hipStream_t stream) {
   if (n_jobs == 0) return;
-  hipLaunchKernelGGL(k_h264_deblock, dim3(n_jobs), dim3(64), 0, stream,
-                     d_curY, d_curCb, d_curCr, ypitch, cpitch, mbw, d_jobs,
-                     d_levels, d_meta);
-}
-
-}
-}
+  hipLaunchKernelGGL(k_h264_deblock, dim3(n_jobs), dim3(128), 0, stream,
+                     d_curY, d_curCb, d_curCr, d_refY, d_refCb, d_refCr,
+                     ypitch, cpitch, mbw, d_jobs, d_levels, d_meta);
+}
+
+}
+}
diff --git a/native/hip/h264_kernels.h b/native/hip/h264_kernels.h
--- a/native/hip/h264_kernels.h
+++ b/native/hip/h264_kernels.h
@@ -33,11 +33,12 @@
                       const RowJob* d_jobs, int16_t* d_levels, int* d_meta,
                       hipStream_t stream);
 
-void launch_h264_deblock(uint8_t* d_curY, uint8_t* d_curCb,
-                         uint8_t* d_curCr, int ypitch, int cpitch, int mbw,
-                         int n_jobs, const RowJob* d_jobs,
-                         const int16_t* d_levels, const int* d_meta,
-                         hipStream_t stream);
+void launch_h264_deblock(const uint8_t* d_curY, const uint8_t* d_curCb,
+                         const uint8_t* d_curCr, uint8_t* d_refY,
+                         uint8_t* d_refCb, uint8_t* d_refCr, int ypitch,
+                         int cpitch, int mbw, int n_jobs,
+                         const RowJob* d_jobs, const int16_t* d_levels,
+                         const int* d_meta, hipStream_t stream);
 
 void launch_h264_rows4_mono(const uint8_t* src, const uint8_t* ref,
                             uint8_t* cur, size_t plane_stride, int pitch,
@@ -45,8 +46,9 @@
                             const RowJob* d_jobs, int16_t* d_levels,
                             int* d_meta, hipStream_t stream);
 
-void launch_h264_deblock_mono(uint8_t* d_cur, size_t plane_stride, int pitch,
-                              int mbw, int n_jobs, const RowJob* d_jobs,
+void launch_h264_deblock_mono(const uint8_t* d_cur, uint8_t* d_ref,
+                              size_t plane_stride, int pitch, int mbw,
+                              int n_jobs, const RowJob* d_jobs,
                               const int* d_meta, hipStream_t stream);
 
 void launch_h264_cavlc_mono(const int16_t* d_levels, const int* d_meta,
diff --git a/native/module.cpp b/native/module.cpp
--- a/native/module.cpp
+++ b/native/module.cpp
@@ -6,8 +6,10 @@
 #include "audio.h"
 #include "cpu/damage.h"
 #include "cpu/h264/cavlc.h"
+#include "cpu/h264/deblock_lines.h"
 #include "cpu/h264/encoder.h"
 #include "cpu/h264/seg_plan.h"
+#include "cpu/h264/transform.h"
 #include "cpu/hevc/cabac.h"
 #include "cpu/hevc/encoder.h"
 #include "cpu/opus/celt.h"
@@ -480,7 +482,8 @@
       "_pipeline_encode",
       [](const std::string& kind, py::list frames, int w, int h, int qp,
          int stripe_h, int output_mode, bool dump, bool fullcolor,
-         int pipeline_depth, py::object encode_mask) -> py::object {
+         int pipeline_depth, py::object encode_mask,
+         bool deblock) -> py::object {
         const size_t n_stripes =
             stripe_h > 0 ? static_cast<size_t>((h + stripe_h - 1) / stripe_h)
                          : 0;
@@ -511,6 +514,7 @@
         s.video_crf = qp;
         s.jpeg_quality = qp;
         s.video_fullcolor = fullcolor;
+        s.video_deblock = deblock;
         s.use_cpu = kind == "cpu";
         s.gpu_id = kind == "cpu" ? -1 : 0;
         std::unique_ptr<EncodePipeline> p;
@@ -585,9 +589,61 @@
       py::arg("qp") = 26, py::arg("stripe_h") = 64,
       py::arg("output_mode") = 1, py::arg("dump") = false,
       py::arg("fullcolor") = false, py::arg("pipeline_depth") = 1,
-      py::arg("encode_mask") = py::none(),
+      py::arg("encode_mask") = py::none(), py::arg("deblock") = true,
       "Test hook: run frames through a named encode pipeline. "
-      "encode_mask[frame][stripe] (optional) gates which stripes encode.");
+      "encode_mask[frame][stripe] (optional) gates which stripes encode; "
+      "deblock=False switches the in-loop filter off (video_deblock).");
+
+  m.def(
+      "_h264_deblock_segment",
+      [](py::buffer y, py::object cb, py::object cr, py::list mbs, int qp,
+         bool lines) -> py::tuple {
+        const int segw = static_cast<int>(mbs.size());
+        auto plane = [](py::buffer b, size_t want) {
+          py::buffer_info info = b.request();
+          if (static_cast<size_t>(info.size * info.itemsize) != want)
+            throw py::value_error("plane size does not match the MB count");
+          const uint8_t* p = static_cast<const uint8_t*>(info.ptr);
+          return std::vector<uint8_t>(p, p + want);
+        };
+        if (segw < 1) throw py::value_error("need at least one MB");
+        if (cb.is_none() != cr.is_none())
+          throw py::value_error("cb and cr go together");
+        const bool mono = cb.is_none();
+        std::vector<uint8_t> Y = plane(y, static_cast<size_t>(segw) * 256);
+        std::vector<uint8_t> Cb, Cr;
+        if (!mono) {
+          Cb = plane(cb.cast<py::buffer>(), static_cast<size_t>(segw) * 64);
+          Cr = plane(cr.cast<py::buffer>(), static_cast<size_t>(segw) * 64);
+        }
+        std::vector<h264::DbMb> info(segw);
+        for (int i = 0; i < segw; ++i) {
+          py::tuple t = mbs[i].cast<py::tuple>();
+          if (t.size() != 4)
+            throw py::value_error("MB info is (intra, mvx, mvy, nz)");
+          info[i].intra = t[0].cast<bool>() ? 1 : 0;
+          info[i].mvx = t[1].cast<int16_t>();
+          info[i].mvy = t[2].cast<int16_t>();
+          info[i].nz = t[3].cast<uint16_t>();
+        }
+        (lines ? h264::deblock_segment_lines : h264::deblock_segment)(
+            Y.data(), segw * 16, mono ? nullptr : Cb.data(),
+            mono ? nullptr : Cr.data(), segw * 8, 0, 0, segw, info.data(),
+            qp, h264::chroma_qp(std::min(51, std::max(0, qp))));
+        auto out = [](const std::vector<uint8_t>& v) {
+          return py::bytes(reinterpret_cast<const char*>(v.data()),
+                           v.size());
+        };
+        if (mono) return py::make_tuple(out(Y));
+        return py::make_tuple(out(Y), out(Cb), out(Cr));
+      },
+      py::arg("y"), py::arg("cb"), py::arg("cr"), py::arg("mbs"),
+      py::arg("qp"), py::arg("lines") = false,
+      "Test hook: deblock one slice segment held in caller-supplied planes "
+      "(luma 16 x 16n, chroma 8 x 8n or None for monochrome) with per-MB "
+      "(intra, mvx, mvy, nz). lines=False runs the scalar reference "
+      "deblock_segment, lines=True the walk in the HIP kernel's order "
+      "(deblock_segment_lines). Returns the filtered planes.");
 
   struct BenchPipeline {
     std::unique_ptr<EncodePipeline> p;
diff --git a/native/pipeline_hip_h264.cpp b/native/pipeline_hip_h264.cpp
--- a/native/pipeline_hip_h264.cpp
+++ b/native/pipeline_hip_h264.cpp
@@ -178,17 +178,16 @@
     }
     HIP_CHECK(hipEventRecord(ev_rows_[par], rows_stream_));
     if (settings_.video_deblock) {
-      HIP_CHECK(hipStreamWaitEvent(db_stream_, ev_rows_[par], 0));
       if (fc_)
-        h264gpu::launch_h264_deblock_mono(d_curY_, plane_stride_, ypitch_,
-                                          mbw_, n_jobs, d_jobs_[par],
-                                          d_meta_[par], db_stream_);
+        h264gpu::launch_h264_deblock_mono(d_curY_, d_refY_, plane_stride_,
+                                          ypitch_, mbw_, n_jobs, d_jobs_[par],
+                                          d_meta_[par], rows_stream_);
       else
-        h264gpu::launch_h264_deblock(d_curY_, d_curCb_, d_curCr_, ypitch_,
-                                     cpitch_, mbw_, n_jobs, d_jobs_[par],
+        h264gpu::launch_h264_deblock(d_curY_, d_curCb_, d_curCr_, d_refY_,
+                                     d_refCb_, d_refCr_, ypitch_, cpitch_,
+                                     mbw_, n_jobs, d_jobs_[par],
                                      d_levels_[par], d_meta_[par],
-                                     db_stream_);
-      HIP_CHECK(hipEventRecord(ev_db_[par], db_stream_));
+                                     rows_stream_);
     }
     int copy_words = 0;
     if (!cpu_entropy_) {
@@ -203,9 +202,7 @@
                                sizeof(int) * n_jobs, hipMemcpyDeviceToHost,
                                stream_));
     }
-    if (settings_.video_deblock)
-      HIP_CHECK(hipStreamWaitEvent(rows_stream_, ev_db_[par], 0));
-    {
+    if (!settings_.video_deblock) {
       int span_y0 = -1, span_y1 = -1;
       auto flush_span = [&] {
         if (span_y0 < 0) return;
@@ -468,7 +465,6 @@
     prev_.active = false;
     stream_.sync();
     up_stream_.sync();
-    db_stream_.sync();
     rows_stream_.sync();
     arena_.release();
     w_ = h_ = 0;
@@ -547,8 +543,8 @@
   UseDevice dev_;
   Arena arena_;
   FrameUploader uploader_;
-  Stream stream_, up_stream_, db_stream_, rows_stream_;
-  Event ev_done_[2], ev_h2d_[2], ev_rows_[2], ev_db_[2];
+  Stream stream_, up_stream_, rows_stream_;
+  Event ev_done_[2], ev_h2d_[2], ev_rows_[2];
   CompactReadback<uint32_t> readback_;
   int stripe_h_ = 64;
   const bool fc_ = settings_.video_fullcolor;
```
